# SHI-Labs/Versatile-Diffusion

Hardware: NVIDIA H100
Metric: 512x512 images/sec @ 50-step DDIM (bs=4/GPU) (higher is better)
Workload: dtype bf16

## Files before the change

### include/vdb200.h

```cpp
#ifndef VDB200_H_
#define VDB200_H_

#include <stddef.h>

#ifdef __cplusplus
extern "C" {
#endif

enum { VDB_OK = 0, VDB_ERR_INVALID = 1, VDB_ERR_CUDA = 2, VDB_ERR_UNSUPPORTED = 3 };
enum { VDB_ACT_NONE = 0, VDB_ACT_SILU = 1, VDB_ACT_GELU = 2, VDB_ACT_QUICK_GELU = 3, VDB_ACT_GEGLU = 4,
       VDB_ACT_GELU_TANH = 5 ,
       VDB_ACT_TANH = 6  };

const char* vdb_version(void);
const char* vdb_last_error(void);
long long vdb_launch_count(void);
void vdb_reset_launch_count(void);
int vdb_num_sms(void);

int vdb_ddim_cfg_step(const float* e_uncond, const float* e_cond, const float* x, const float* noise,
                      const float* coef, const int* step_idx, float scale, float temperature, float* x_prev,
                      float* x_prev_dup, float* pred_x0, long long n, void* stream);
int vdb_axpby_f32(const float* x, const float* z, float a, float b, float* y, long long n, void* stream);
int vdb_add_int(int* p, int delta, void* stream);
int vdb_lincomb4_f32(const float* x0, const float* x1, const float* x2, const float* x3, float c0, float c1, float c2,
                     float c3, float* y, long long n, void* stream);

int vdb_gemm_bf16(const void* A, long long M, long long K, long long lda, const void* A2, long long K2,
                  long long lda2, const void* W, long long N, long long ldw, const float* bias,
                  long long bias_bstride, long long rows_per_batch, const void* resid, long long ldr, void* out,
                  long long ldo, int out_f32, int act, float alpha, int bn, int ksplit, void* workspace,
                  size_t ws_bytes, void* stream);

int vdb_igemm_last_plan(int* out, int n);

int vdb_gemm_ln_bf16(const void* A, long long M, long long K, long long lda, const void* W, long long N, long long ldw,
                     const float* bias, const void* resid, long long ldr, void* out, long long ldo, int act,
                     const float* ln_stats, long long ln_rows, int ln_parts, int ln_dim, float ln_eps, const float* ln_colsum,
                     int ln_on_cols, const float* ln_rowbias, float* stats_out, int* stats_parts, int bn, void* stream);

int vdb_gemm_skinny_fits(int S, long long K);
int vdb_gemm_skinny_bf16(const void* small1, int S, long long K1, long long lds1, const void* small2, long long K2, long long lds2,
                         const void* big, long long R, long long ldb, const float* bias, long long bias_bstride,
                         const void* resid, long long ldr, void* out, long long ldo, int transpose_out, void* stream);

int vdb_conv3x3_bf16(const void* X, int B, int H, int W, int C, int mode, const void* Wt, int N, long long ldw,
                     const void* skip1, int Cs1, const void* skip2, int Cs2, const float* bias,
                     long long bias_bstride, const void* resid, long long ldr, void* out, long long ldo,
                     int out_f32, int act, int bn, int ksplit, void* workspace, size_t ws_bytes, void* stream);

int vdb_attention_dk_pad(int d_head);
int vdb_attention_dv_pad(int d_head);
int vdb_attention_bf16(const void* Q, long long ldq, int q_col0, const void* K, long long ldk, int k_col0,
                       const void* Vt, long long ldv, void* out, long long ldo, int B, int H, int Nq, int Nk,
                       int q_bstride, int kv_bstride, int d_head, float scale, int causal, void* stream);
int vdb_attention_varlen_bf16(const void* Q, long long ldq, int q_col0, const void* K, long long ldk, int k_col0,
                              const void* Vt, long long ldv, void* out, long long ldo, int B, int H, int Nq, int Nk,
                              int q_bstride, int kv_bstride, int d_head, float scale, int causal, const int* kv_len,
                              void* stream);

int vdb_groupnorm_nsplit(int B, int HW);
long long vdb_groupnorm_scratch_floats(int B, int HW);
int vdb_groupnorm_nhwc(const void* x1, int C1, const void* x2, int C2, int B, int HW, int groups, const float* gamma,
                       const float* beta, float eps, int act, float* scratch, void* y, void* stream);

int vdb_layernorm(const void* x, long long rows, int C, const float* gamma, const float* beta, float eps, void* y,
                  void* stream);

int vdb_norm_last_plan(int* out, int n);

int vdb_upsample2x_nhwc(const void* x, int B, int H, int W, int C, void* y, void* stream);

int vdb_clip_to_u8_hwc(const float* x, int n, int H, int W, void* y , void* stream);
int vdb_resample_h_u8(const void* x , int n, int H, int Win, int Wout, const int* bounds, const int* kk,
                      int ksize, void* y , void* stream);
int vdb_resample_v_crop_norm(const void* x , int n, int Hin, int W, const int* bounds, const int* kk,
                             int ksize , int top, int left, int S, const float* mean3,
                             const float* std3, float* y , void* stream);

int vdb_interleave2x2_nhwc(const void* src, int B, int H, int W, int C, void* y, void* stream);

int vdb_im2col3x3_small(const float* x, int B, int H, int W, int Cin, int Kpad, float in_scale, float in_shift,
                        void* y, void* stream);

int vdb_permute_f32(const float* x, int B, int C, long long HW, int to_nhwc, float mul, float add, int clamp01,
                    float* y, void* stream);
int vdb_gaussian_sample(const float* moments, const float* noise, int C, long long npix, float post_mul, float* z,
                        void* stream);
int vdb_cast_f32_bf16(const float* x, void* y, long long n, void* stream);
int vdb_pointwise_small(const float* x, long long npix, int Cin, int Cout, const float* Wm, const float* bias,
                        float pre_mul, float* y, void* stream);
int vdb_cast_bf16_f32(const void* x, float* y, long long n, void* stream);

int vdb_timestep_embedding(const long long* ts, const int* step_idx, int B, int dim, float neg_log_period,
                           float* out, void* stream);

int vdb_linear_small(const float* x, int M, int K, const void* Wt, int N, const float* bias, int act_in, int act_out,
                     float* out, void* stream);

int vdb_clip_text_embed(const long long* tokens, const float* tok_emb, const float* pos_emb, int B, int L, int Lp, int C,
                        void* x, void* stream);
int vdb_patchify(const float* pixels, int B, int Cin, int HW, int P, int Kpad, void* y, void* stream);
int vdb_vit_assemble(const void* patches, const float* cls, const float* pos, const float* tok_scale, int B, int L, int Lp,
                     int C, void* x, void* stream);
int vdb_scale_by_row_norm(const void* z, const int* idx, const float* row_scale, int B, int L, int Lp, int C, float* out,
                          void* stream);

int vdb_softmax_rows(const void* x, long long rows, int n, long long ld, float scale, void* y, void* stream);

int vdb_affine_act_rows(const void* x, long long rows, int n, const float* gamma, const float* beta, int act, void* y, void* stream);

int vdb_pack_conv_weight(const float* w, int Cout, int Cin, int kh, int kw, void* out, long long ldo, long long col0, void* stream);
int vdb_pack_geglu(const float* w, const float* b, int n2, int K, void* w_out, float* b_out, void* stream);
int vdb_pad_heads(const float* w, int H, int d, int dpad, int K, void* out, void* stream);

int vdb_textdec_gemv(const float* x, int R, long long K, long long ldx, const float* ln_gamma, const float* ln_beta, float ln_eps,
                     const void* W, long long N, long long ldw, const float* bias, int act, int accumulate, float* out, long long ldo,
                     void* stream);
int vdb_textdec_attention(const float* qkv, long long ldq, const float* mem, long long ldm, float* kcache, float* vcache, int R,
                          int H, int T, const int* step, float scale, float* out, long long ldo, void* stream);
int vdb_textdec_embed(const int* tokens, int ldt, const int* step, const float* wte, int V, const float* wpe, int P, int pos_offset,
                      const float* emb, int R, int D, float* h, void* stream);
int vdb_textdec_sample(const float* logits, int R, int V, long long ldl, float temperature, const unsigned long long* seed,
                       const double* uniforms, int ldu, const int* forced, int ldf, int* tokens, int ldt, int* done, int* lengths,
                       const int* step, int eos, int max_len, float* record, void* stream);

#ifdef __cplusplus
}
#endif
#endif
```

### versatile-diffusion_b200/csrc/common.cuh

```cuda
#pragma once
#include <cuda.h>
#include <cuda_bf16.h>
#include <cuda_runtime.h>
#include <stdint.h>

namespace vdb {

#define VDB_DEVINL __device__ __forceinline__

enum : int {
  VDB_OK = 0,
  VDB_ERR_INVALID = 1,
  VDB_ERR_CUDA = 2,
  VDB_ERR_UNSUPPORTED = 3,
};

VDB_DEVINL float4 lds_f4(uint32_t addr) {
  float4 v;
  asm volatile("ld.shared.v4.f32 {%0, %1, %2, %3}, [%4];" : "=f"(v.x), "=f"(v.y), "=f"(v.z), "=f"(v.w) : "r"(addr));
  return v;
}

VDB_DEVINL float2 lds_f2(uint32_t addr) {
  float2 v;
  asm volatile("ld.shared.v2.f32 {%0, %1}, [%2];" : "=f"(v.x), "=f"(v.y) : "r"(addr));
  return v;
}
VDB_DEVINL void stmatrix_x4(uint32_t addr, uint32_t r0, uint32_t r1, uint32_t r2, uint32_t r3) {
  asm volatile("stmatrix.sync.aligned.m8n8.x4.shared.b16 [%0], {%1, %2, %3, %4};" ::"r"(addr), "r"(r0), "r"(r1), "r"(r2), "r"(r3)
               : "memory");
}

VDB_DEVINL uint32_t smem_u32(const void* p) {
  return static_cast<uint32_t>(__cvta_generic_to_shared(p));
}

VDB_DEVINL uint32_t lane_id() {
  uint32_t l;
  asm volatile("mov.u32 %0, %%laneid;" : "=r"(l));
  return l;
}

VDB_DEVINL bool elect_one() {
  uint32_t pred = 0;
  asm volatile(
      "{\n\t"
      ".reg .pred P;\n\t"
      "elect.sync _|P, 0xffffffff;\n\t"
      "selp.u32 %0, 1, 0, P;\n\t"
      "}\n"
      : "=r"(pred));
  return pred != 0;
}

VDB_DEVINL void mbar_init(uint64_t* bar, uint32_t count) {
  asm volatile("mbarrier.init.shared::cta.b64 [%0], %1;" ::"r"(smem_u32(bar)), "r"(count));
}
VDB_DEVINL void fence_barrier_init() {
  asm volatile("fence.mbarrier_init.release.cluster;" ::: "memory");
}
VDB_DEVINL void fence_proxy_async_smem() {
  asm volatile("fence.proxy.async.shared::cta;" ::: "memory");
}
VDB_DEVINL void mbar_arrive_expect_tx(uint64_t* bar, uint32_t bytes) {
  asm volatile("mbarrier.arrive.expect_tx.shared::cta.b64 _, [%0], %1;" ::"r"(smem_u32(bar)),
               "r"(bytes)
               : "memory");
}
VDB_DEVINL void mbar_arrive(uint64_t* bar) {
  asm volatile("mbarrier.arrive.shared::cta.b64 _, [%0];" ::"r"(smem_u32(bar)) : "memory");
}
VDB_DEVINL bool mbar_try_wait(uint64_t* bar, uint32_t parity) {
  uint32_t ok;
  asm volatile(
      "{\n\t"
      ".reg .pred P;\n\t"
      "mbarrier.try_wait.parity.shared::cta.b64 P, [%1], %2;\n\t"
      "selp.u32 %0, 1, 0, P;\n\t"
      "}\n"
      : "=r"(ok)
      : "r"(smem_u32(bar)), "r"(parity)
      : "memory");
  return ok != 0;
}
VDB_DEVINL void mbar_wait(uint64_t* bar, uint32_t parity) {
  while (!mbar_try_wait(bar, parity)) {
  }
}

VDB_DEVINL void tma_prefetch_desc(const CUtensorMap* m) {
  asm volatile("prefetch.tensormap [%0];" ::"l"(reinterpret_cast<uint64_t>(m)) : "memory");
}
VDB_DEVINL void tma_load_2d(void* smem_dst, const CUtensorMap* m, uint64_t* bar, int c0, int c1) {
  asm volatile(
      "cp.async.bulk.tensor.2d.shared::cluster.global.tile.mbarrier::complete_tx::bytes"
      " [%0], [%1, {%3, %4}], [%2];" ::"r"(smem_u32(smem_dst)),
      "l"(reinterpret_cast<uint64_t>(m)), "r"(smem_u32(bar)), "r"(c0), "r"(c1)
      : "memory");
}
VDB_DEVINL void tma_load_4d(void* smem_dst, const CUtensorMap* m, uint64_t* bar, int c0, int c1,
                            int c2, int c3) {
  asm volatile(
      "cp.async.bulk.tensor.4d.shared::cluster.global.tile.mbarrier::complete_tx::bytes"
      " [%0], [%1, {%3, %4, %5, %6}], [%2];" ::"r"(smem_u32(smem_dst)),
      "l"(reinterpret_cast<uint64_t>(m)), "r"(smem_u32(bar)), "r"(c0), "r"(c1), "r"(c2), "r"(c3)
      : "memory");
}

VDB_DEVINL void tma_store_4d(const CUtensorMap* m, const void* smem_src, int c0, int c1, int c2, int c3) {
  asm volatile(
      "cp.async.bulk.tensor.4d.global.shared::cta.tile.bulk_group [%0, {%2, %3, %4, %5}], [%1];" ::"l"(
          reinterpret_cast<uint64_t>(m)),
      "r"(smem_u32(smem_src)), "r"(c0), "r"(c1), "r"(c2), "r"(c3)
      : "memory");
}
VDB_DEVINL void bulk_commit() { asm volatile("cp.async.bulk.commit_group;" ::: "memory"); }
template <int N>
VDB_DEVINL void bulk_wait_read() { asm volatile("cp.async.bulk.wait_group.read %0;" ::"n"(N) : "memory"); }
template <int N>
VDB_DEVINL void bulk_wait() { asm volatile("cp.async.bulk.wait_group %0;" ::"n"(N) : "memory"); }

VDB_DEVINL uint32_t cluster_ctarank() {
  uint32_t r;
  asm volatile("mov.u32 %0, %%cluster_ctarank;" : "=r"(r));
  return r;
}
VDB_DEVINL void cluster_sync_all() {
  asm volatile("barrier.cluster.arrive.release.aligned;\n\tbarrier.cluster.wait.acquire.aligned;" ::: "memory");
}
VDB_DEVINL uint32_t mapa_u32(uint32_t local_addr, uint32_t rank) {
  uint32_t r;
  asm volatile("mapa.shared::cluster.u32 %0, %1, %2;" : "=r"(r) : "r"(local_addr), "r"(rank));
  return r;
}
VDB_DEVINL void mbar_arrive_cluster(uint32_t cluster_addr) {
  asm volatile("mbarrier.arrive.release.cluster.shared::cluster.b64 _, [%0];" ::"r"(cluster_addr) : "memory");
}

VDB_DEVINL uint64_t make_desc_sw128(uint32_t smem_addr) {
  uint64_t d = 0;
  d |= static_cast<uint64_t>((smem_addr & 0x3FFFF) >> 4);
  d |= static_cast<uint64_t>(1) << 16;
  d |= static_cast<uint64_t>(1024 >> 4) << 32;
  d |= static_cast<uint64_t>(1) << 62;
  return d;
}
VDB_DEVINL void wgmma_fence() { asm volatile("wgmma.fence.sync.aligned;" ::: "memory"); }
VDB_DEVINL void wgmma_commit() { asm volatile("wgmma.commit_group.sync.aligned;" ::: "memory"); }
template <int N>
VDB_DEVINL void wgmma_wait() { asm volatile("wgmma.wait_group.sync.aligned %0;" ::"n"(N) : "memory"); }
template <int R>
VDB_DEVINL void wgmma_fence_regs(float (&d)[R]) {
#pragma unroll
  for (int i = 0; i < R; ++i) asm volatile("" : "+f"(d[i])::"memory");
}

VDB_DEVINL unsigned long long gtime() {
  unsigned long long t;
  asm volatile("mov.u64 %0, %%globaltimer;" : "=l"(t));
  return t;
}

VDB_DEVINL void pdl_wait() { asm volatile("griddepcontrol.wait;" ::: "memory"); }
VDB_DEVINL void pdl_launch_dependents() { asm volatile("griddepcontrol.launch_dependents;" ::: "memory"); }

VDB_DEVINL uint32_t pack_bf16x2(float lo, float hi) {
  __nv_bfloat162 v = __floats2bfloat162_rn(lo, hi);
  return *reinterpret_cast<uint32_t*>(&v);
}
VDB_DEVINL float2 unpack_bf16x2(uint32_t u) {
  __nv_bfloat162 v = *reinterpret_cast<__nv_bfloat162*>(&u);
  return __bfloat1622float2(v);
}
VDB_DEVINL float ex2_mufu(float x) {
  float y;
  asm("ex2.approx.ftz.f32 %0, %1;" : "=f"(y) : "f"(x));
  return y;
}
VDB_DEVINL float ex2_poly(float x) {
  x = fmaxf(x, -126.0f);
  const float r = x + 12582912.0f;
  const float f = x - (r - 12582912.0f);
  float p = fmaf(0.0550886838f, f, 0.242604051f);
  p = fmaf(p, f, 0.693276242f);
  p = fmaf(p, f, 0.99992894f);
  return __int_as_float(__float_as_int(p) + (__float_as_int(r) << 23));
}
VDB_DEVINL float silu_f(float x) { return __fdividef(x, 1.0f + __expf(-x)); }
VDB_DEVINL float silu_bf16_f(float x) {
  float th;
  asm("tanh.approx.f32 %0, %1;" : "=f"(th) : "f"(0.5f * x));
  const float hx = 0.5f * x;
  return fmaf(hx, th, hx);
}
VDB_DEVINL float gelu_erf_f(float x) { return 0.5f * x * (1.0f + erff(x * 0.70710678118654752f)); }
VDB_DEVINL float gelu_as_f(float x) {
  const float z = fabsf(x) * 0.70710678118654752f;
  const float t = __fdividef(1.0f, fmaf(0.3275911f, z, 1.0f));
  float poly = fmaf(1.061405429f, t, -1.453152027f);
  poly = fmaf(poly, t, 1.421413741f);
  poly = fmaf(poly, t, -0.284496736f);
  poly = fmaf(poly, t, 0.254829592f);
  const float erf_abs = 1.0f - poly * t * __expf(-z * z);
  return 0.5f * x * (1.0f + copysignf(erf_abs, x));
}
VDB_DEVINL float gelu_fast_f(float x) {
  const float u = x * fmaf(0.0356774081f, x * x, 0.7978845608f);
  float th;
  asm("tanh.approx.f32 %0, %1;" : "=f"(th) : "f"(u));
  const float hx = 0.5f * x;
  return fmaf(hx, th, hx);
}
VDB_DEVINL float quick_gelu_f(float x) { return __fdividef(x, 1.0f + __expf(-1.702f * x)); }

}

#include "wgmma.cuh"
```

### versatile-diffusion_b200/csrc/igemm.cu

```cuda
#include "common.cuh"
#include "host_util.h"

namespace vdb {

constexpr int kBlockM = 128;
constexpr int kBlockK = 64;
constexpr int kMaxA = 6;
constexpr int kMaxSeg = 12;
constexpr uint32_t kABytes = kBlockM * kBlockK * 2;

struct ASeg {
  int16_t tmap;
  int16_t dw;
  int16_t dh;
  int16_t nkb;
  int32_t c0;
};

struct alignas(64) IgemmParams {
  CUtensorMap tmA[kMaxA];
  CUtensorMap tmB;
  CUtensorMap tmO;
  ASeg seg[kMaxSeg];
  int nseg;
  int kb_total;
  int ksplit;
  int kb_per_split;
  int TW, TH, TB;
  int Wo, Ho, Bo;
  int tilesW, tilesH, tilesB, tilesN;
  int N;
  const float* bias;
  long long bias_bstride;
  int rows_per_batch;
  const __nv_bfloat16* resid;
  long long ldr;
  void* out;
  long long ldo;
  int out_f32;
  int act;
  float alpha;
  float* partial;
  const float* ln_stats;
  long long ln_mstat;
  int ln_parts;
  int ln_on_cols;
  float ln_inv_dim, ln_eps;
  const float* ln_colsum;
  const float* ln_rowbias;
  float* stats_out;
  int epi_alt;
  int nfast;
  unsigned long long* timeline;
  unsigned smem_bytes;
  int chunked;
};

enum { ACT_NONE = 0, ACT_SILU = 1, ACT_GELU = 2, ACT_QGELU = 3, ACT_GEGLU = 4 };

#ifdef VDB_TIMELINE
#define VDB_TL(slot, it) do { if (p.timeline && blockIdx.x == 0 && (it) < 8) p.timeline[(it) * 16 + (slot)] = gtime(); } while (0)
#define VDB_TLE(slot, it) do { if (warp == 0 && lane == 0) VDB_TL(slot, it); } while (0)
#else
#define VDB_TL(slot, it) do { } while (0)
#define VDB_TLE(slot, it) do { } while (0)
#endif

VDB_DEVINL float apply_act(float v, int act) {
  switch (act) {
    case ACT_SILU: return silu_f(v);
    case ACT_GELU: return gelu_erf_f(v);
    case ACT_QGELU: return quick_gelu_f(v);
    default: return v;
  }
}

template <int BN, int STAGES, int EW, int MODE>
__global__ void __launch_bounds__(32 + 32 * EW, 1) igemm_kernel(const __grid_constant__ IgemmParams p) {
  constexpr bool kTmaEpi = MODE >= 3;
  constexpr bool kGegluEpi = MODE == 4 || MODE == 6;
  constexpr bool kLnIn = MODE == 5 || MODE == 6;
  constexpr bool kStatsOut = MODE == 7;
  constexpr int kNumEpiWarps = EW;
  constexpr int kNumEpiThreads = EW * 32;
  constexpr int kWPQ = EW / 4;
  static_assert(EW == 8, "two consumer warpgroups of 64 rows each");
  constexpr uint32_t kBBytes = BN * kBlockK * 2;
  constexpr uint32_t kStageBytes = kABytes + kBBytes;
  constexpr int kAccStride = BN + 4;
  constexpr uint32_t kRingBytes = STAGES * kStageBytes;
  constexpr uint32_t kAccBytes = kBlockM * kAccStride * 4;
  constexpr uint32_t kRegion = kRingBytes > kAccBytes ? kRingBytes : kAccBytes;
  static_assert(kBBytes % 1024 == 0, "B stage must keep 1024B alignment");
  static_assert(BN % 32 == 0 && BN >= 32 && BN <= 256, "invalid wgmma N");

  extern __shared__ __align__(1024) uint8_t smem_raw[];
  uint8_t* smem = reinterpret_cast<uint8_t*>((reinterpret_cast<uintptr_t>(smem_raw) + 1023) & ~uintptr_t(1023));
  uint8_t* smemA = smem;
  uint8_t* smemB = smem + STAGES * kABytes;
  float* sacc = reinterpret_cast<float*>(smem);
  float* sstage = reinterpret_cast<float*>(smem + kRegion);
  uint64_t* full_bar = reinterpret_cast<uint64_t*>(smem + kRegion + EW * 4096);
  uint64_t* empty_bar = full_bar + STAGES;
  uint64_t* acc_free = empty_bar + STAGES;
  float* sbias = reinterpret_cast<float*>(acc_free + 2);
  float* slnx = sbias + BN;
  const uint32_t sbias_s = smem_u32(sbias), slnx_s = smem_u32(slnx);
  (void)slnx_s;
  if constexpr (kLnIn) {
    if (reinterpret_cast<uint8_t*>(slnx + BN) > smem_raw + p.smem_bytes) __trap();
  }
  auto epi_bar_sync = [] { asm volatile("bar.sync 1, %0;" ::"n"(EW * 32) : "memory"); };

  const int warp = threadIdx.x >> 5;
  const int lane = threadIdx.x & 31;

  if (warp == EW && lane == 0) {
    for (int i = 0; i < kMaxA; ++i) tma_prefetch_desc(&p.tmA[i]);
    tma_prefetch_desc(&p.tmB);
    if constexpr (MODE >= 3) tma_prefetch_desc(&p.tmO);
  }
  if (threadIdx.x == 0) {
    for (int s = 0; s < STAGES; ++s) {
      mbar_init(&full_bar[s], 1);
      mbar_init(&empty_bar[s], kNumEpiWarps);
    }
    mbar_init(acc_free, kNumEpiWarps);
    fence_barrier_init();
  }
  __syncthreads();
  pdl_launch_dependents();
  pdl_wait();

  const int tilesM = p.tilesW * p.tilesH * p.tilesB;
  const int unitsM = tilesM;
  const int num_tiles = unitsM * p.tilesN * p.ksplit;
  const int n_ctas = gridDim.x, cta_id = blockIdx.x;
  const int per_cta = (num_tiles + n_ctas - 1) / n_ctas;
  const int t_first = p.chunked ? cta_id * per_cta : cta_id, t_step = p.chunked ? 1 : n_ctas;
  const int t_end = p.chunked ? min(num_tiles, t_first + per_cta) : num_tiles;

  if (warp == EW) {
    if (lane == 0) {
      uint32_t stage = 0, phase = 0;
      const bool flat = (p.tilesH == 1) && (p.tilesB == 1);
      const int step_m = t_step % unitsM, step_r = t_step / unitsM;
      int unit_m = t_first % unitsM, rest = t_first / unitsM;
      const int nf_step_n = p.nfast ? t_step % p.tilesN : 0, nf_step_m = p.nfast ? t_step / p.tilesN : 0;
      int nf_n = p.nfast ? t_first % p.tilesN : 0, nf_m = p.nfast ? t_first / p.tilesN : 0;
      int it = 0;
      for (int t = t_first; t < t_end; t += t_step, ++it) {
        const int m_idx = p.nfast ? nf_m : unit_m;
        int n_idx = p.nfast ? nf_n : rest, ks = 0;
        if (p.ksplit > 1) { n_idx = rest % p.tilesN; ks = rest / p.tilesN; }
        nf_n += nf_step_n; nf_m += nf_step_m;
        if (p.nfast && nf_n >= p.tilesN) { nf_n -= p.tilesN; ++nf_m; }
        int wt = m_idx, ht = 0, bt = 0;
        if (!flat) {
          wt = m_idx % p.tilesW;
          const int q = m_idx / p.tilesW;
          ht = q % p.tilesH;
          bt = q / p.tilesH;
        }
        unit_m += step_m; rest += step_r;
        if (unit_m >= unitsM) { unit_m -= unitsM; ++rest; }
        const int w0 = wt * p.TW, h0 = ht * p.TH, b0 = bt * p.TB;
        const int n0 = n_idx * BN;
        const int kb_begin = ks * p.kb_per_split;
        const int kb_end = min(p.kb_total, kb_begin + p.kb_per_split);
        int kb = 0;
        if (!kTmaEpi && it > 0) mbar_wait(acc_free, (it - 1) & 1);
        VDB_TL(0, it);
        for (int s = 0; s < p.nseg; ++s) {
          const ASeg sg = p.seg[s];
          if (kb + sg.nkb <= kb_begin) { kb += sg.nkb; continue; }
          for (int j = 0; j < sg.nkb; ++j, ++kb) {
            if (kb < kb_begin) continue;
            if (kb >= kb_end) break;
            mbar_wait(&empty_bar[stage], phase ^ 1);
            mbar_arrive_expect_tx(&full_bar[stage], kStageBytes);
            tma_load_4d(smemA + stage * kABytes, &p.tmA[sg.tmap], &full_bar[stage],
                        sg.c0 + j * kBlockK, w0 + sg.dw, h0 + sg.dh, b0);
            tma_load_2d(smemB + stage * kBBytes, &p.tmB, &full_bar[stage], kb * kBlockK, n0);
            if (++stage == STAGES) { stage = 0; phase ^= 1; }
          }
          if (kb >= kb_end) break;
        }
      }
    }
  } else {
    const int quarter = warp & 3;
    const int half = warp >> 2;
    const int r = quarter * 32 + lane;
    const int tr_row = lane >> 2, tr_q = lane & 3;
    float* stage = sstage + warp * 1024;
    const uint32_t sacc_row = smem_u32(sacc) + static_cast<uint32_t>(r * kAccStride * 4);
    auto acc_ld32 = [&](int col, uint32_t (&v)[32]) {
#pragma unroll
      for (int i = 0; i < 8; ++i) {
        const float4 x = lds_f4(sacc_row + (col + 4 * i) * 4);
        v[4 * i] = __float_as_uint(x.x); v[4 * i + 1] = __float_as_uint(x.y);
        v[4 * i + 2] = __float_as_uint(x.z); v[4 * i + 3] = __float_as_uint(x.w);
      }
    };
    uint32_t ml_stage = 0, ml_phase = 0;
    float acc[BN / 2];
    auto mainloop = [&](int kb_begin, int kb_end) {
      const int g = warp >> 2;
#pragma unroll
      for (int i = 0; i < BN / 2; ++i) acc[i] = 0.f;
      uint32_t prev = 0;
      for (int kb = kb_begin; kb < kb_end; ++kb) {
        mbar_wait(&full_bar[ml_stage], ml_phase);
        wgmma_fence();
        const uint64_t adesc = make_desc_sw128(smem_u32(smemA + ml_stage * kABytes + g * (64 * 128)));
        const uint64_t bdesc = make_desc_sw128(smem_u32(smemB + ml_stage * kBBytes));
#pragma unroll
        for (int k = 0; k < kBlockK / 16; ++k) wgmma_ss<BN>(acc, adesc + 2 * k, bdesc + 2 * k, (kb > kb_begin || k > 0) ? 1u : 0u);
        wgmma_commit();
        if (kb > kb_begin) {
          wgmma_wait<1>();
          __syncwarp();
          if (lane == 0) mbar_arrive(&empty_bar[prev]);
        }
        prev = ml_stage;
        if (++ml_stage == STAGES) { ml_stage = 0; ml_phase ^= 1; }
      }
      wgmma_wait<0>();
      wgmma_fence_regs(acc);
      __syncwarp();
      if (lane == 0 && kb_end > kb_begin) mbar_arrive(&empty_bar[prev]);
      if constexpr (!kTmaEpi) {
        epi_bar_sync();
        float* srow = sacc + (g * 64 + (warp & 3) * 16 + (lane >> 2)) * kAccStride + 2 * (lane & 3);
#pragma unroll
        for (int j = 0; j < BN / 8; ++j) {
          *reinterpret_cast<float2*>(srow + 8 * j) = make_float2(acc[4 * j], acc[4 * j + 1]);
          *reinterpret_cast<float2*>(srow + 8 * kAccStride + 8 * j) = make_float2(acc[4 * j + 2], acc[4 * j + 3]);
        }
        epi_bar_sync();
      }
    };
    auto stage_write = [&](const uint32_t (&v)[32]) {
      float* srow = stage + lane * 32;
#pragma unroll
      for (int j = 0; j < 8; ++j)
        *reinterpret_cast<uint4*>(srow + ((j ^ (lane & 7)) << 2)) = make_uint4(v[4 * j], v[4 * j + 1], v[4 * j + 2], v[4 * j + 3]);
    };
    auto stage_read = [&](int k, float (&o)[8]) {
      const int row = k * 8 + tr_row;
      const float* srow = stage + row * 32;
      const float4 x0 = *reinterpret_cast<const float4*>(srow + (((2 * tr_q) ^ (row & 7)) << 2));
      const float4 x1 = *reinterpret_cast<const float4*>(srow + (((2 * tr_q + 1) ^ (row & 7)) << 2));
      o[0] = x0.x; o[1] = x0.y; o[2] = x0.z; o[3] = x0.w; o[4] = x1.x; o[5] = x1.y; o[6] = x1.z; o[7] = x1.w;
    };
    int it = 0;
    int st_buf = 0;
    (void)st_buf;
    const float* sbias_src = nullptr;
    const int tw = r % p.TW;
    const int th = (r / p.TW) % p.TH;
    const int tb = r / (p.TW * p.TH);
    const bool flat = (p.tilesH == 1) && (p.tilesB == 1);
    const int step_m = t_step % unitsM, step_r = t_step / unitsM;
    int unit_m = t_first % unitsM, rest = t_first / unitsM;
    const int nf_step_n = p.nfast ? t_step % p.tilesN : 0, nf_step_m = p.nfast ? t_step / p.tilesN : 0;
    int nf_n = p.nfast ? t_first % p.tilesN : 0, nf_m = p.nfast ? t_first / p.tilesN : 0;
    const int e_row0 = (warp >> 2) * 64 + (warp & 3) * 16;
    int e_tw[2], e_th[2], e_tb[2];
#pragma unroll
    for (int h = 0; h < 2; ++h) {
      const int er = e_row0 + (lane >> 2) + 8 * h;
      e_tw[h] = er % p.TW; e_th[h] = (er / p.TW) % p.TH; e_tb[h] = er / (p.TW * p.TH);
    }
    constexpr int kLnPre = 8;
    float2 ln_pre[kLnIn ? kLnPre : 1];
    auto ln_prefetch = [&](int row) {
      if constexpr (kLnIn) {
        const bool ok = row < p.Wo;
        const int i0 = (lane >> 4) * kLnPre;
#pragma unroll
        for (int i = 0; i < kLnPre; ++i)
          ln_pre[i] = (ok && i0 + i < p.ln_parts)
                          ? __ldg(reinterpret_cast<const float2*>(p.ln_stats) + static_cast<long long>(i0 + i) * p.ln_mstat + row)
                          : make_float2(0.f, 0.f);
      }
    };
    if constexpr (kLnIn) {
      if (!p.ln_on_cols && p.ln_parts <= 2 * kLnPre && t_first < t_end) ln_prefetch((t_first % unitsM) * kBlockM + e_row0 + (lane & 15));
    }
    for (int t = t_first; t < t_end; t += t_step, ++it) {
      const int m_idx = p.nfast ? nf_m : unit_m;
      int n_idx = p.nfast ? nf_n : rest, ks = 0;
      if (p.ksplit > 1) { n_idx = rest % p.tilesN; ks = rest / p.tilesN; }
      nf_n += nf_step_n; nf_m += nf_step_m;
      if (p.nfast && nf_n >= p.tilesN) { nf_n -= p.tilesN; ++nf_m; }
      int wt = m_idx, ht = 0, bt = 0;
      if (!flat) {
        wt = m_idx % p.tilesW;
        const int q = m_idx / p.tilesW;
        ht = q % p.tilesH;
        bt = q / p.tilesH;
      }
      unit_m += step_m; rest += step_r;
      if (unit_m >= unitsM) { unit_m -= unitsM; ++rest; }
      const int w = wt * p.TW + tw, h = ht * p.TH + th, b = bt * p.TB + tb;
      const bool row_ok = (w < p.Wo) && (h < p.Ho) && (b < p.Bo);
      const int gp = (b * p.Ho + h) * p.Wo + w;
      const int gp_first = ((bt * p.TB) * p.Ho + ht * p.TH) * p.Wo + wt * p.TW;
      const int n0 = n_idx * BN;

      int gp_k[4];
      bool ok_k[4];
      if constexpr (!kTmaEpi) {
        const unsigned okmask = __ballot_sync(0xffffffffu, row_ok);
#pragma unroll
        for (int k = 0; k < 4; ++k) {
          const int src = k * 8 + tr_row;
          gp_k[k] = __shfl_sync(0xffffffffu, gp, src);
          ok_k[k] = (okmask >> src) & 1u;
        }
      }
      const int gp_last = ((bt * p.TB + p.TB - 1) * p.Ho + ht * p.TH + p.TH - 1) * p.Wo + wt * p.TW + p.TW - 1;
      const bool bias_uniform = (MODE != 0) ? (p.bias != nullptr)
                                            : (p.bias && p.ksplit == 1 &&
                                               (p.bias_bstride == 0 || gp_first / p.rows_per_batch == gp_last / p.rows_per_batch));
      if constexpr (kLnIn) {
        const float* key = reinterpret_cast<const float*>(static_cast<uintptr_t>(n0) + 1);
        if (key != sbias_src) {
          epi_bar_sync();
          for (int i = threadIdx.x; i < BN; i += kNumEpiThreads) {
            const int n = n0 + i;
            float a = 0.f, b = 0.f;
            if (n < p.N) {
              if (p.ln_on_cols) {
                float su = 0.f, sq = 0.f;
#pragma unroll 8
                for (int ch = 0; ch < p.ln_parts; ++ch) {
                  const float2 v = __ldg(reinterpret_cast<const float2*>(p.ln_stats) + static_cast<long long>(ch) * p.ln_mstat + n);
                  su += v.x; sq += v.y;
                }
                const float mu = su * p.ln_inv_dim;
                a = mu;
                b = rsqrtf(fmaxf(sq * p.ln_inv_dim - mu * mu, 0.f) + p.ln_eps);
              } else {
                a = __ldg(p.ln_colsum + n);
                b = p.bias ? __ldg(p.bias + n) : 0.f;
              }
            }
            slnx[i] = a;
            sbias[i] = b;
          }
          epi_bar_sync();
          sbias_src = key;
        }
      } else if (bias_uniform) {
        const float* brow = p.bias + (p.bias_bstride ? static_cast<long long>(gp_first / p.rows_per_batch) * p.bias_bstride : 0) + n0;
        if (brow != sbias_src) {
          epi_bar_sync();
          for (int i = threadIdx.x; i < BN; i += kNumEpiThreads) sbias[i] = (n0 + i < p.N) ? __ldg(brow + i) : 0.f;
          epi_bar_sync();
          sbias_src = brow;
        }
      }
      const float* bias_g = (p.bias && !bias_uniform)
                                ? p.bias + (p.bias_bstride ? static_cast<long long>(gp / p.rows_per_batch) * p.bias_bstride : 0) : nullptr;

      const int f_nchunks = min(BN / 32, (p.N - n0) / 32);
      const bool has_resid = p.resid != nullptr;
      const int f_first = (((BN / 32) % kWPQ) != 0) ? ((half + it) % kWPQ) : half;
      auto load_resid_fast = [&](int c, uint4 (&rr)[4]) {
#pragma unroll
        for (int k = 0; k < 4; ++k)
          if (ok_k[k]) rr[k] = __ldg(reinterpret_cast<const uint4*>(p.resid + static_cast<long long>(gp_k[k]) * p.ldr + n0 + c * 32 + tr_q * 8));
      };
      uint4 rr_first[4];
      if constexpr (MODE == 1) {
        if (has_resid && f_first < f_nchunks) load_resid_fast(f_first, rr_first);
      }

      int e_gp[2];
      bool e_ok[2];
#pragma unroll
      for (int h = 0; h < 2; ++h) {
        const int ew = wt * p.TW + e_tw[h], eh = ht * p.TH + e_th[h], eb = bt * p.TB + e_tb[h];
        e_ok[h] = (ew < p.Wo) && (eh < p.Ho) && (eb < p.Bo);
        e_gp[h] = (eb * p.Ho + eh) * p.Wo + ew;
      }
      float ln_a0[2] = {0.f, 0.f}, ln_a1[2] = {1.f, 1.f};
      if constexpr (kLnIn) {
        if (p.ln_on_cols) {
#pragma unroll
          for (int h = 0; h < 2; ++h) {
            if (e_ok[h]) {
              ln_a0[h] = __ldg(p.ln_colsum + e_gp[h]);
              ln_a1[h] = p.ln_rowbias ? __ldg(p.ln_rowbias + e_gp[h]) : 0.f;
            }
          }
        } else {
          float su = 0.f, sq = 0.f;
          if (p.ln_parts <= 2 * kLnPre) {
#pragma unroll
            for (int i = 0; i < kLnPre; ++i) { su += ln_pre[i].x; sq += ln_pre[i].y; }
#pragma unroll
            for (int i = 0; i < kLnPre; ++i) {
              su += __shfl_sync(0xffffffffu, ln_pre[i].x, lane | 16);
              sq += __shfl_sync(0xffffffffu, ln_pre[i].y, lane | 16);
            }
          } else {
            const int row = m_idx * kBlockM + e_row0 + (lane & 15);
            if (row < p.Wo) {
#pragma unroll 8
              for (int ch = 0; ch < p.ln_parts; ++ch) {
                const float2 v = __ldg(reinterpret_cast<const float2*>(p.ln_stats) + static_cast<long long>(ch) * p.ln_mstat + row);
                su += v.x; sq += v.y;
              }
            }
          }
          const float mu = su * p.ln_inv_dim;
          const float rs = rsqrtf(fmaxf(sq * p.ln_inv_dim - mu * mu, 0.f) + p.ln_eps);
#pragma unroll
          for (int h = 0; h < 2; ++h) {
            ln_a0[h] = __shfl_sync(0xffffffffu, mu, (lane >> 2) + 8 * h);
            ln_a1[h] = __shfl_sync(0xffffffffu, rs, (lane >> 2) + 8 * h);
          }
        }
        if (!p.ln_on_cols && p.ln_parts <= 2 * kLnPre && t + t_step < t_end) ln_prefetch(unit_m * kBlockM + e_row0 + (lane & 15));
      }
      VDB_TLE(4, it);
      mainloop(ks * p.kb_per_split, min(p.kb_total, ks * p.kb_per_split + p.kb_per_split));
      VDB_TLE(5, it);

      auto geglu_tile = [&] {
        constexpr int HALF = BN / 2;
        const int nout0 = n_idx * HALF;
        const int Nout = p.N / 2;
#pragma unroll 1
        for (int c = (((HALF / 32) % kWPQ) != 0) ? ((half + it) % kWPQ) : half; c < HALF / 32; c += kWPQ) {
          uint32_t v[32];
          float a[4][8];
          acc_ld32(c * 32, v);
          stage_write(v);
          __syncwarp();
#pragma unroll
          for (int k = 0; k < 4; ++k) stage_read(k, a[k]);
          __syncwarp();
          acc_ld32(HALF + c * 32, v);
          stage_write(v);
          __syncwarp();
          float bv[8], bg[8];
#pragma unroll
          for (int i = 0; i < 8; ++i) {
            bv[i] = p.bias ? sbias[c * 32 + tr_q * 8 + i] : 0.f;
            bg[i] = p.bias ? sbias[HALF + c * 32 + tr_q * 8 + i] : 0.f;
          }
#pragma unroll
          for (int k = 0; k < 4; ++k) {
            float g[8];
            stage_read(k, g);
            if (ok_k[k] && nout0 + c * 32 + tr_q * 8 + 7 < Nout) {
              float o[8];
#pragma unroll
              for (int i = 0; i < 8; ++i) o[i] = (a[k][i] + bv[i]) * gelu_fast_f(g[i] + bg[i]);
              *reinterpret_cast<uint4*>(reinterpret_cast<__nv_bfloat16*>(p.out) + static_cast<long long>(gp_k[k]) * p.ldo + nout0 + c * 32 + tr_q * 8) =
                  make_uint4(pack_bf16x2(o[0], o[1]), pack_bf16x2(o[2], o[3]), pack_bf16x2(o[4], o[5]), pack_bf16x2(o[6], o[7]));
            }
          }
          __syncwarp();
        }
      };
      if constexpr (kTmaEpi) {
        const uint32_t stg_s = smem_u32(sstage) + warp * 4096;
        const int ow = wt * p.TW + (e_row0 % p.TW), oh = ht * p.TH + ((e_row0 / p.TW) % p.TH), ob = bt * p.TB + e_row0 / (p.TW * p.TH);
        constexpr int OUTC = kGegluEpi ? BN / 2 : BN;
        const int ochunks = kGegluEpi ? OUTC / 32 : f_nchunks;
        const int ocol0 = n_idx * OUTC;
        const int tq2 = 2 * (lane & 3);
        const bool do_resid = (MODE == 3 || MODE == 7) && has_resid;
        const uint32_t* rrow[2];
#pragma unroll
        for (int h = 0; h < 2; ++h)
          rrow[h] = (do_resid && e_ok[h]) ? reinterpret_cast<const uint32_t*>(p.resid + static_cast<long long>(e_gp[h]) * p.ldr + ocol0 + tq2)
                                          : nullptr;
        auto load_resid = [&](int c, uint32_t (&rr)[2][4]) {
#pragma unroll
          for (int h = 0; h < 2; ++h)
#pragma unroll
            for (int jj = 0; jj < 4; ++jj) rr[h][jj] = rrow[h] ? __ldg(rrow[h] + (c * 32 + 8 * jj) / 2) : 0u;
        };
        uint32_t rr[2][4];
        if (do_resid) load_resid(0, rr);
        float st_su[2][2] = {{0.f, 0.f}, {0.f, 0.f}}, st_sq[2][2] = {{0.f, 0.f}, {0.f, 0.f}};
        (void)st_su; (void)st_sq;
        float nrm[2];
#pragma unroll
        for (int h = 0; h < 2; ++h) nrm[h] = -ln_a1[h] * ln_a0[h];
        (void)nrm;
#pragma unroll
        for (int c = 0; c < OUTC / 32; ++c) {
          if (c >= ochunks) break;
          float o[4][2][2];
#pragma unroll
          for (int jj = 0; jj < 4; ++jj) {
            const int n = c * 32 + 8 * jj + tq2;
            const float* va = acc + 4 * (4 * c + jj);
            if constexpr (kGegluEpi) {
              const float* vg = acc + 4 * (BN / 16 + 4 * c + jj);
              if constexpr (kLnIn) {
                const float2 sa = lds_f2(slnx_s + 4 * n), ca = lds_f2(sbias_s + 4 * n);
                const float2 sg = lds_f2(slnx_s + 4 * (OUTC + n)), cg = lds_f2(sbias_s + 4 * (OUTC + n));
#pragma unroll
                for (int h = 0; h < 2; ++h) {
                  o[jj][h][0] = fmaf(ln_a1[h], va[2 * h], fmaf(nrm[h], sa.x, ca.x)) * gelu_fast_f(fmaf(ln_a1[h], vg[2 * h], fmaf(nrm[h], sg.x, cg.x)));
                  o[jj][h][1] = fmaf(ln_a1[h], va[2 * h + 1], fmaf(nrm[h], sa.y, ca.y)) * gelu_fast_f(fmaf(ln_a1[h], vg[2 * h + 1], fmaf(nrm[h], sg.y, cg.y)));
                }
              } else {
                const float2 ba = p.bias ? lds_f2(sbias_s + 4 * n) : make_float2(0.f, 0.f);
                const float2 bg = p.bias ? lds_f2(sbias_s + 4 * (OUTC + n)) : make_float2(0.f, 0.f);
#pragma unroll
                for (int h = 0; h < 2; ++h) {
                  o[jj][h][0] = (va[2 * h] + ba.x) * gelu_fast_f(vg[2 * h] + bg.x);
                  o[jj][h][1] = (va[2 * h + 1] + ba.y) * gelu_fast_f(vg[2 * h + 1] + bg.y);
                }
              }
            } else if constexpr (kLnIn) {
              if (p.ln_on_cols) {
                const float2 mu = lds_f2(slnx_s + 4 * n), rs = lds_f2(sbias_s + 4 * n);
#pragma unroll
                for (int h = 0; h < 2; ++h) {
                  o[jj][h][0] = fmaf(rs.x, fmaf(mu.x, -ln_a0[h], va[2 * h]), ln_a1[h]);
                  o[jj][h][1] = fmaf(rs.y, fmaf(mu.y, -ln_a0[h], va[2 * h + 1]), ln_a1[h]);
                }
              } else {
                const float2 sx = lds_f2(slnx_s + 4 * n), cx = lds_f2(sbias_s + 4 * n);
#pragma unroll
                for (int h = 0; h < 2; ++h) {
                  o[jj][h][0] = fmaf(ln_a1[h], va[2 * h], fmaf(nrm[h], sx.x, cx.x));
                  o[jj][h][1] = fmaf(ln_a1[h], va[2 * h + 1], fmaf(nrm[h], sx.y, cx.y));
                }
              }
            } else {
              const float2 bb = p.bias ? lds_f2(sbias_s + 4 * n) : make_float2(0.f, 0.f);
#pragma unroll
              for (int h = 0; h < 2; ++h) {
                o[jj][h][0] = va[2 * h] + bb.x;
                o[jj][h][1] = va[2 * h + 1] + bb.y;
              }
            }
          }
          if (do_resid) {
            uint32_t rn[2][4];
            const bool more = c + 1 < ochunks;
            if (more) load_resid(c + 1, rn);
#pragma unroll
            for (int h = 0; h < 2; ++h)
#pragma unroll
              for (int jj = 0; jj < 4; ++jj) {
                const float2 x = unpack_bf16x2(rr[h][jj]);
                o[jj][h][0] += x.x;
                o[jj][h][1] += x.y;
              }
            if (more) {
#pragma unroll
              for (int h = 0; h < 2; ++h)
#pragma unroll
                for (int jj = 0; jj < 4; ++jj) rr[h][jj] = rn[h][jj];
            }
          }
          if constexpr (kStatsOut) {
#pragma unroll
            for (int h = 0; h < 2; ++h)
#pragma unroll
              for (int jj = 0; jj < 4; ++jj)
#pragma unroll
                for (int e = 0; e < 2; ++e) {
                  st_su[h][c & 1] += o[jj][h][e];
                  st_sq[h][c & 1] = fmaf(o[jj][h][e], o[jj][h][e], st_sq[h][c & 1]);
                }
          }
          if (lane == 0) bulk_wait_read<3>();
          __syncwarp();
          const uint32_t box = stg_s + st_buf * 1024;
          {
            const int mi = lane >> 3, brow = (mi & 1) * 8 + (lane & 7);
#pragma unroll
            for (int u = 0; u < 2; ++u) {
              const int unit = 2 * u + (mi >> 1);
              stmatrix_x4(box + brow * 64 + ((unit ^ ((brow >> 1) & 3)) << 4),
                          pack_bf16x2(o[2 * u][0][0], o[2 * u][0][1]), pack_bf16x2(o[2 * u][1][0], o[2 * u][1][1]),
                          pack_bf16x2(o[2 * u + 1][0][0], o[2 * u + 1][0][1]), pack_bf16x2(o[2 * u + 1][1][0], o[2 * u + 1][1][1]));
            }
          }
          fence_proxy_async_smem();
          __syncwarp();
          if (lane == 0) {
            tma_store_4d(&p.tmO, reinterpret_cast<const uint8_t*>(sstage) + warp * 4096 + st_buf * 1024, ocol0 + c * 32, ow, oh, ob);
            bulk_commit();
          }
          st_buf = (st_buf + 1) & 3;
        }
        if constexpr (kStatsOut) {
#pragma unroll
          for (int h = 0; h < 2; ++h)
#pragma unroll
            for (int par = 0; par < 2; ++par) {
              float su = st_su[h][par], sq = st_sq[h][par];
              su += __shfl_xor_sync(0xffffffffu, su, 1); sq += __shfl_xor_sync(0xffffffffu, sq, 1);
              su += __shfl_xor_sync(0xffffffffu, su, 2); sq += __shfl_xor_sync(0xffffffffu, sq, 2);
              if ((lane & 3) == 0 && e_ok[h])
                reinterpret_cast<float2*>(p.stats_out)[static_cast<long long>(n_idx * 2 + par) * (static_cast<long long>(p.Bo) * p.Ho * p.Wo) + e_gp[h]] =
                    make_float2(su, sq);
            }
        }
      } else if constexpr (MODE == 1) {
        uint4 rr[4];
#pragma unroll
        for (int k = 0; k < 4; ++k) rr[k] = rr_first[k];
#pragma unroll 1
        for (int c = f_first; c < f_nchunks; c += kWPQ) {
          uint32_t v[32];
          acc_ld32(c * 32, v);
          uint4 rn[4];
          if (has_resid && c + kWPQ < f_nchunks) load_resid_fast(c + kWPQ, rn);
          stage_write(v);
          __syncwarp();
          float bb[8];
#pragma unroll
          for (int i = 0; i < 8; ++i) bb[i] = p.bias ? sbias[c * 32 + tr_q * 8 + i] : 0.f;
#pragma unroll
          for (int k = 0; k < 4; ++k) {
            float o[8];
            stage_read(k, o);
            if (ok_k[k]) {
#pragma unroll
              for (int i = 0; i < 8; ++i) o[i] += bb[i];
              if (has_resid) {
                const uint32_t w4[4] = {rr[k].x, rr[k].y, rr[k].z, rr[k].w};
#pragma unroll
                for (int q = 0; q < 4; ++q) {
                  const float2 x = unpack_bf16x2(w4[q]);
                  o[2 * q] += x.x;
                  o[2 * q + 1] += x.y;
                }
              }
              *reinterpret_cast<uint4*>(reinterpret_cast<__nv_bfloat16*>(p.out) + static_cast<long long>(gp_k[k]) * p.ldo + n0 + c * 32 + tr_q * 8) =
                  make_uint4(pack_bf16x2(o[0], o[1]), pack_bf16x2(o[2], o[3]), pack_bf16x2(o[4], o[5]), pack_bf16x2(o[6], o[7]));
            }
          }
          __syncwarp();
#pragma unroll
          for (int k = 0; k < 4; ++k) rr[k] = rn[k];
        }
      } else if constexpr (MODE == 2) {
        geglu_tile();
      } else if (p.ksplit > 1) {
        const long long Mtot = static_cast<long long>(p.Bo) * p.Ho * p.Wo;
        float* dst = p.partial + (static_cast<long long>(ks) * Mtot + gp) * p.N + n0;
#pragma unroll 1
        for (int c = half; c < BN / 32; c += kWPQ) {
          if (n0 + c * 32 >= p.N) break;
          uint32_t v[32];
          acc_ld32(c * 32, v);
          if (row_ok) {
#pragma unroll
            for (int j = 0; j < 32; j += 4) {
              const int n = n0 + c * 32 + j;
              if (n + 3 < p.N) {
                *reinterpret_cast<float4*>(dst + c * 32 + j) =
                    make_float4(__uint_as_float(v[j]), __uint_as_float(v[j + 1]),
                                __uint_as_float(v[j + 2]), __uint_as_float(v[j + 3]));
              } else {
                for (int q = 0; q < 4; ++q)
                  if (n + q < p.N) dst[c * 32 + j + q] = __uint_as_float(v[j + q]);
              }
            }
          }
        }
      } else if (p.act == ACT_GEGLU) {
        geglu_tile();
      } else {
        const int nchunks = min(BN / 32, (p.N - n0 + 31) / 32);
        auto chunk = [&](int c, const uint32_t (&v)[32], const uint4 (&rr)[4], bool fast) {
          const int nb = n0 + c * 32;
          if (fast) {
            stage_write(v);
            __syncwarp();
            if (c == half) VDB_TLE(8, it);
            float bb[8];
#pragma unroll
            for (int i = 0; i < 8; ++i) bb[i] = p.bias ? sbias[c * 32 + tr_q * 8 + i] : 0.f;
#pragma unroll
            for (int k = 0; k < 4; ++k) {
              float o[8];
              stage_read(k, o);
              if (ok_k[k]) {
#pragma unroll
                for (int i = 0; i < 8; ++i) o[i] += bb[i];
                if (p.alpha != 1.f) {
#pragma unroll
                  for (int i = 0; i < 8; ++i) o[i] *= p.alpha;
                }
                if (p.act != ACT_NONE) {
#pragma unroll
                  for (int i = 0; i < 8; ++i) o[i] = apply_act(o[i], p.act);
                }
                if (p.resid) {
                  const uint32_t w4[4] = {rr[k].x, rr[k].y, rr[k].z, rr[k].w};
#pragma unroll
                  for (int q = 0; q < 4; ++q) {
                    const float2 x = unpack_bf16x2(w4[q]);
                    o[2 * q] += x.x;
                    o[2 * q + 1] += x.y;
                  }
                }
                *reinterpret_cast<uint4*>(reinterpret_cast<__nv_bfloat16*>(p.out) + static_cast<long long>(gp_k[k]) * p.ldo + nb + tr_q * 8) =
                    make_uint4(pack_bf16x2(o[0], o[1]), pack_bf16x2(o[2], o[3]), pack_bf16x2(o[4], o[5]), pack_bf16x2(o[6], o[7]));
              }
              if (c == half && k == 0) VDB_TLE(9, it);
            }
            __syncwarp();
            if (c == half) VDB_TLE(10, it);
          } else if (row_ok) {
            float f[32];
#pragma unroll
            for (int j = 0; j < 32; ++j) f[j] = __uint_as_float(v[j]);
            if (p.bias) {
#pragma unroll
              for (int j = 0; j < 32; ++j)
                if (nb + j < p.N) f[j] += bias_uniform ? sbias[c * 32 + j] : __ldg(bias_g + nb + j);
            }
#pragma unroll
            for (int j = 0; j < 32; ++j) f[j] = apply_act(f[j] * p.alpha, p.act);
            if (p.resid) {
              const __nv_bfloat16* rs = p.resid + static_cast<long long>(gp) * p.ldr + nb;
#pragma unroll
              for (int j = 0; j < 32; ++j) if (nb + j < p.N) f[j] += __bfloat162float(rs[j]);
            }
            if (p.out_f32) {
              float* dst = reinterpret_cast<float*>(p.out) + static_cast<long long>(gp) * p.ldo + nb;
#pragma unroll
              for (int j = 0; j < 32; ++j) if (nb + j < p.N) dst[j] = f[j];
            } else {
              __nv_bfloat16* dst = reinterpret_cast<__nv_bfloat16*>(p.out) + static_cast<long long>(gp) * p.ldo + nb;
#pragma unroll
              for (int j = 0; j < 32; ++j) if (nb + j < p.N) dst[j] = __float2bfloat16(f[j]);
            }
          }
        };
        auto is_fast = [&](int c) { return (n0 + c * 32 + 32 <= p.N) && !p.out_f32 && (bias_uniform || !p.bias); };
        auto load_resid = [&](int c, uint4 (&rr)[4]) {
          if (p.resid && is_fast(c)) {
#pragma unroll
            for (int k = 0; k < 4; ++k)
              if (ok_k[k]) rr[k] = __ldg(reinterpret_cast<const uint4*>(p.resid + static_cast<long long>(gp_k[k]) * p.ldr + n0 + c * 32 + tr_q * 8));
          }
        };
        const int first = (p.epi_alt && ((BN / 32) % kWPQ) != 0) ? ((half + it) % kWPQ) : half;
#pragma unroll 1
        for (int c = first; c < nchunks; c += kWPQ) {
          uint4 rr[4];
          load_resid(c, rr);
          uint32_t v[32];
          acc_ld32(c * 32, v);
          if (c == first) VDB_TLE(7, it);
          chunk(c, v, rr, is_fast(c));
        }
      }
      if constexpr (!kTmaEpi) {
        fence_proxy_async_smem();
        __syncwarp();
        VDB_TLE(6, it);
        if (lane == 0) mbar_arrive(acc_free);
      }
    }
    if constexpr (MODE >= 3) {
      if (lane == 0) bulk_wait<0>();
    }
  }
}

__global__ void splitk_reduce_kernel(const float* __restrict__ partial, int ksplit, long long M, int N,
                                     const float* __restrict__ bias, long long bias_bstride, int rows_per_batch,
                                     const __nv_bfloat16* __restrict__ resid, long long ldr, void* out,
                                     long long ldo, int out_f32, int act, float alpha) {
  pdl_launch_dependents();
  pdl_wait();
  const long long total = M * (N / 4);
  for (long long i = blockIdx.x * static_cast<long long>(blockDim.x) + threadIdx.x; i < total;
       i += static_cast<long long>(gridDim.x) * blockDim.x) {
    const long long m = i / (N / 4);
    const int n = static_cast<int>(i % (N / 4)) * 4;
    float4 acc = make_float4(0.f, 0.f, 0.f, 0.f);
    for (int s = 0; s < ksplit; ++s) {
      const float4 v = __ldg(reinterpret_cast<const float4*>(partial + (static_cast<long long>(s) * M + m) * N + n));
      acc.x += v.x; acc.y += v.y; acc.z += v.z; acc.w += v.w;
    }
    float f[4] = {acc.x, acc.y, acc.z, acc.w};
    if (bias) {
      const float* bp = bias + (bias_bstride ? (m / rows_per_batch) * bias_bstride : 0) + n;
      for (int q = 0; q < 4; ++q) f[q] += __ldg(bp + q);
    }
    for (int q = 0; q < 4; ++q) f[q] *= alpha;
    for (int q = 0; q < 4; ++q) f[q] = apply_act(f[q], act);
    if (resid) {
      for (int q = 0; q < 4; ++q) f[q] += __bfloat162float(resid[m * ldr + n + q]);
    }
    if (out_f32) {
      *reinterpret_cast<float4*>(reinterpret_cast<float*>(out) + m * ldo + n) = make_float4(f[0], f[1], f[2], f[3]);
    } else {
      uint2 o = make_uint2(pack_bf16x2(f[0], f[1]), pack_bf16x2(f[2], f[3]));
      *reinterpret_cast<uint2*>(reinterpret_cast<__nv_bfloat16*>(out) + m * ldo + n) = o;
    }
  }
}

template <int BN, int STAGES, int EW, int MODE>
static int launch_igemm(const IgemmParams& p0, int num_units, cudaStream_t stream) {
  constexpr bool kLn = MODE == 5 || MODE == 6;
  constexpr size_t ring = STAGES * (kABytes + BN * kBlockK * 2), acc = kBlockM * (BN + 4) * 4;
  constexpr size_t need = (ring > acc ? ring : acc) + (2 * STAGES + 2) * 8 + BN * 4 + (kLn ? BN * 4 : 0) + EW * 4096;
  constexpr size_t smem = (need + 1024 <= 227 * 1024) ? need + 1024 : 227 * 1024;
  static_assert(need + 896 <= 227 * 1024, "igemm shared-memory budget");
  constexpr int threads = 32 + 32 * EW;
  IgemmParams p = p0;
  p.smem_bytes = static_cast<unsigned>(smem);
  static bool configured = false;
  if (!configured) {
    VDB_CUDA_CHECK(cudaFuncSetAttribute(igemm_kernel<BN, STAGES, EW, MODE>, cudaFuncAttributeMaxDynamicSharedMemorySize,
                                        static_cast<int>(smem)));
    prefer_max_smem(igemm_kernel<BN, STAGES, EW, MODE>);
    configured = true;
  }
  const int grid = std::min(num_units, num_sms());
  VDB_CUDA_CHECK(launch_pdl(igemm_kernel<BN, STAGES, EW, MODE>, dim3(grid), dim3(threads), smem, stream, p));
  count_launch();
  return VDB_OK;
}

static int pick_bn(int N, int act, int forced) {
  if (forced) return forced;
  if (act == ACT_GEGLU) return 256;
  if (N <= 64) return 64;
  if (N % 256 == 0) return 256;
  if (N % 160 == 0) return 160;
  if (N % 128 == 0) return 128;
  if (N <= 128) return 128;
  if (N <= 160) return 160;
  return 256;
}

static unsigned long long* g_timeline = nullptr;

constexpr int kPlanFields = 9;
static thread_local int g_last_plan[kPlanFields] = {0};

static int check_epilogue_pointers(const void* out, long long ldo, int out_f32, const void* resid, long long ldr, const char* who) {
  if ((reinterpret_cast<uintptr_t>(out) & 15) || (resid && (reinterpret_cast<uintptr_t>(resid) & 15)))
    return set_error(VDB_ERR_INVALID, "%s: out and resid must be 16-byte aligned", who);
  if (!out_f32 && (ldo % 8)) return set_error(VDB_ERR_INVALID, "%s: ldo must be a multiple of 8 for bf16 out", who);
  if (resid && (ldr % 8)) return set_error(VDB_ERR_INVALID, "%s: ldr must be a multiple of 8", who);
  return VDB_OK;
}

struct IgemmEpilogue {
  const float* bias = nullptr;
  long long bias_bstride = 0;
  int rows_per_batch = 1;
  const void* resid = nullptr;
  long long ldr = 0;
  void* out = nullptr;
  long long ldo = 0;
  int out_f32 = 0;
  int act = 0;
  float alpha = 1.f;
  const float* ln_stats = nullptr;
  long long ln_mstat = 0;
  int ln_parts = 0;
  int ln_dim = 0;
  float ln_eps = 0.f;
  const float* ln_colsum = nullptr;
  int ln_on_cols = 0;
  const float* ln_rowbias = nullptr;
  float* stats_out = nullptr;
  int* stats_parts = nullptr;
  int out_parity = -1;
};

static int run_igemm(IgemmParams& p, const void* Wt, long long N, long long Ktot, long long ldw,
                     const IgemmEpilogue& e, int bn_forced, int ksplit_forced, void* workspace,
                     size_t ws_bytes, cudaStream_t stream) {
  const bool ln_in = e.ln_stats != nullptr, st_out = e.stats_out != nullptr;
  if (ln_in || st_out) ksplit_forced = 1;
  int BN = pick_bn(static_cast<int>(N), e.act, bn_forced);
  static const int bn_model = [] { const char* ev = getenv("VDB_BN_MODEL"); return (ev && ev[0] == '0') ? 0 : 1; }();
  if (bn_model && !bn_forced && e.act != ACT_GEGLU && p.kb_total >= 8) {
    const long long tm = static_cast<long long>(p.tilesW) * p.tilesH * p.tilesB;
    const int cand[4] = {256, 160, 128, 64};
    double best = 1e30;
    for (int c : cand) {
      const long long tiles = tm * ((N + c - 1) / c);
      long long ks = 1;
      if (ksplit_forced > 0) ks = ksplit_forced;
      else if (tiles * 2 <= num_sms() && p.kb_total >= 16 && (N % 4) == 0 && workspace)
        ks = std::max<long long>(1, std::min<long long>(std::min<long long>(num_sms() / tiles, p.kb_total / 8), 16));
      const long long waves = (tiles * ks + num_sms() - 1) / num_sms();
      const double per_kb = std::max(2.0 * c, (16384.0 + 128.0 * c) / 90.0);
      const double kb_unit = static_cast<double>((p.kb_total + ks - 1) / ks);
      const double cost = static_cast<double>(waves) * (kb_unit * per_kb + 1500.0) + (ks > 1 ? 12000.0 : 0.0);
      if (cost < best * 0.97) { best = cost; BN = c; }
    }
  }
  if (!bn_forced && !bn_model && e.act != ACT_GEGLU && p.kb_total < 32) {
    const int tm = p.tilesW * p.tilesH * p.tilesB;
    auto tiles = [&](int bn) { return tm * static_cast<int>((N + bn - 1) / bn); };
    while (BN > 64 && tiles(BN) * 2 <= num_sms()) BN = (BN == 256) ? 160 : (BN == 160 ? 128 : 64);
  }
  if (BN != 64 && BN != 128 && BN != 160 && BN != 256) return set_error(VDB_ERR_INVALID, "igemm: bad BN");
  if (e.act == ACT_GEGLU && (N % BN) != 0) return set_error(VDB_ERR_INVALID, "igemm: GEGLU needs N % 256 == 0");
  p.N = static_cast<int>(N);
  p.tilesN = static_cast<int>((N + BN - 1) / BN);
  p.bias = e.bias; p.bias_bstride = e.bias_bstride; p.rows_per_batch = e.rows_per_batch > 0 ? e.rows_per_batch : 1;
  p.resid = reinterpret_cast<const __nv_bfloat16*>(e.resid); p.ldr = e.ldr;
  p.out = e.out; p.ldo = e.ldo; p.out_f32 = e.out_f32; p.act = e.act; p.alpha = e.alpha;
  const long long M = static_cast<long long>(p.Bo) * p.Ho * p.Wo;
  if (M >= (1LL << 30)) return set_error(VDB_ERR_UNSUPPORTED, "igemm: more than 2^30 output rows");
  const int tilesM = p.tilesW * p.tilesH * p.tilesB;
  const int mn_tiles = tilesM * p.tilesN;
  int ksplit = 1;
  if (ksplit_forced > 0) {
    ksplit = ksplit_forced;
  } else if (e.act != ACT_GEGLU && mn_tiles * 2 <= num_sms() && p.kb_total >= 16 && (N % 4) == 0) {
    ksplit = std::min(std::min(num_sms() / mn_tiles, p.kb_total / 8), 16);
    if (ksplit < 1) ksplit = 1;
  }
  if (ksplit > 1) {
    const size_t need = static_cast<size_t>(ksplit) * M * N * sizeof(float);
    if (workspace == nullptr || ws_bytes < need || e.act == ACT_GEGLU || (N % 4) || (e.out_f32 && (e.ldo % 4))) ksplit = 1;
  }
  p.ksplit = ksplit;
  p.kb_per_split = (p.kb_total + ksplit - 1) / ksplit;
  p.ksplit = (p.kb_total + p.kb_per_split - 1) / p.kb_per_split;
  p.partial = reinterpret_cast<float*>(workspace);
  p.ln_stats = e.ln_stats; p.ln_mstat = e.ln_mstat; p.ln_parts = e.ln_parts; p.ln_on_cols = e.ln_on_cols;
  if (e.stats_parts) *e.stats_parts = 2 * p.tilesN;
  p.ln_inv_dim = e.ln_dim > 0 ? 1.f / static_cast<float>(e.ln_dim) : 0.f; p.ln_eps = e.ln_eps;
  p.ln_colsum = e.ln_colsum; p.ln_rowbias = e.ln_rowbias; p.stats_out = e.stats_out;
  p.timeline = g_timeline;
  static const int epi_alt = [] { const char* ev = getenv("VDB_EPI_ALT"); return (ev && ev[0] == '0') ? 0 : 1; }();
  p.epi_alt = epi_alt;
  static const int nfast_mode = [] { const char* ev = getenv("VDB_NFAST"); return ev ? atoi(ev) : 0; }();
  {
    const int grid = std::min(mn_tiles * p.ksplit, num_sms());
    const double a_bytes = static_cast<double>(M) * static_cast<double>(Ktot) * 2.0;
    p.nfast = (nfast_mode != 0 && p.ksplit == 1 && p.tilesN > 1 && (grid % p.tilesN) == 0 &&
               (nfast_mode == 2 || a_bytes > 48e6) && !ln_in) ? 1 : 0;
  }
  {
    static const int chunked_mode = [] { const char* ev = getenv("VDB_CHUNKED"); return ev ? atoi(ev) : 0; }();
    const long long units = static_cast<long long>(tilesM) * p.tilesN * p.ksplit;
    const int grid = static_cast<int>(std::min<long long>(units, num_sms()));
    p.chunked = (chunked_mode != 0 && !p.nfast && p.ksplit == 1 && p.tilesN > 1 && units >= 3LL * grid) ? 1 : 0;
  }
  int rc = make_tmap_2d(&p.tmB, Wt, static_cast<uint64_t>(Ktot), static_cast<uint64_t>(N),
                        static_cast<uint64_t>(ldw) * 2, kBlockK, BN);
  if (rc) return rc;
  const int num_tiles = mn_tiles * p.ksplit;
  static const int spec = [] { const char* ev = getenv("VDB_IGEMM_SPEC"); return (ev && ev[0] == '0') ? 0 : 1; }();
  int mode = 0;
  const bool one_bias_row = e.bias == nullptr || e.bias_bstride == 0 ||
                            (p.TB == 1 && (static_cast<long long>(p.Ho) * p.Wo == p.rows_per_batch ||
                                           (p.Ho == 1 && p.Bo == 1 && p.rows_per_batch % kBlockM == 0)));
  if (spec && p.ksplit == 1 && !e.out_f32 && one_bias_row) {
    if (e.act == ACT_GEGLU && BN == 256) mode = 2;
    else if (e.act == ACT_NONE && e.alpha == 1.f && (N % 32) == 0) mode = 1;
  }
  static const int epi_tma = [] { const char* ev = getenv("VDB_EPI_TMA"); return (ev && ev[0] == '0') ? 0 : 1; }();
  if (epi_tma && (mode == 1 || mode == 2) && (reinterpret_cast<uintptr_t>(e.out) & 15) == 0 &&
      (!e.resid || (reinterpret_cast<uintptr_t>(e.resid) & 15) == 0)) {
    const int bw = std::min(p.TW, 16), bh = std::min(p.TH, 16 / bw), bb = 16 / (bw * bh);
    const long long ncols = (mode == 2) ? N / 2 : N;
    const int py = e.out_parity >= 0 ? (e.out_parity >> 1) : 0, px = e.out_parity >= 0 ? (e.out_parity & 1) : 0;
    const uint64_t il = e.out_parity >= 0 ? 2 : 1;
    const void* obase = reinterpret_cast<const __nv_bfloat16*>(e.out) + (static_cast<long long>(py) * (il * p.Wo) + px) * e.ldo;
    if (bb <= p.TB &&
        make_tmap_4d_sw64(&p.tmO, obase, static_cast<uint64_t>(ncols), static_cast<uint64_t>(p.Wo), static_cast<uint64_t>(p.Ho),
                          static_cast<uint64_t>(p.Bo), il * static_cast<uint64_t>(e.ldo) * 2,
                          il * il * static_cast<uint64_t>(p.Wo) * e.ldo * 2,
                          il * il * static_cast<uint64_t>(p.Ho) * p.Wo * e.ldo * 2, 32, bw, bh, bb) == 0)
      mode += 2;
  }
  if (e.out_parity >= 0 && mode != 3)
    return set_error(VDB_ERR_UNSUPPORTED, "igemm: the interleaved-output upsample modes need the TMA-store epilogue (bf16 out, no "
                                          "activation, N %% 32 == 0, aligned out, VDB_EPI_TMA != 0)");
  if (ln_in || st_out) {
    if (ln_in && st_out) return set_error(VDB_ERR_UNSUPPORTED, "igemm: a launch either consumes or produces LayerNorm statistics");
    if (mode != 3 && !(mode == 4 && ln_in))
      return set_error(VDB_ERR_UNSUPPORTED, "igemm: LayerNorm statistics need the TMA-store epilogue (bf16 out, no activation or "
                                            "GEGLU, alpha 1, N %% 32 == 0, 16-byte aligned out / resid, VDB_EPI_TMA != 0)");
    if (ln_in && e.resid) return set_error(VDB_ERR_UNSUPPORTED, "igemm: a folded-LayerNorm GEMM takes no residual");
    if (ln_in && mode == 4 && e.ln_on_cols) return set_error(VDB_ERR_UNSUPPORTED, "igemm: GEGLU with column statistics");
    mode = st_out ? 7 : mode + 2;
  }
  {
    const int stages = BN == 64 ? 8 : BN == 128 ? 6 : BN == 160 ? 5 : 4;
    const int plan[kPlanFields] = {BN, stages, mode, p.ksplit, std::min(num_tiles, num_sms()), tilesM, p.tilesN, p.nfast, p.chunked};
    for (int i = 0; i < kPlanFields; ++i) g_last_plan[i] = plan[i];
  }
  if (mode == 7) {
    switch (BN) {
      case 64: rc = launch_igemm<64, 8, 8, 7>(p, num_tiles, stream); break;
      case 128: rc = launch_igemm<128, 6, 8, 7>(p, num_tiles, stream); break;
      case 160: rc = launch_igemm<160, 5, 8, 7>(p, num_tiles, stream); break;
      default: rc = launch_igemm<256, 4, 8, 7>(p, num_tiles, stream); break;
    }
  } else if (mode == 6) {
    rc = launch_igemm<256, 4, 8, 6>(p, num_tiles, stream);
  } else if (mode == 5) {
    switch (BN) {
      case 64: rc = launch_igemm<64, 8, 8, 5>(p, num_tiles, stream); break;
      case 128: rc = launch_igemm<128, 6, 8, 5>(p, num_tiles, stream); break;
      case 160: rc = launch_igemm<160, 5, 8, 5>(p, num_tiles, stream); break;
      default: rc = launch_igemm<256, 4, 8, 5>(p, num_tiles, stream); break;
    }
  } else if (mode == 4) {
    rc = launch_igemm<256, 4, 8, 4>(p, num_tiles, stream);
  } else if (mode == 3) {
    switch (BN) {
      case 64: rc = launch_igemm<64, 8, 8, 3>(p, num_tiles, stream); break;
      case 128: rc = launch_igemm<128, 6, 8, 3>(p, num_tiles, stream); break;
      case 160: rc = launch_igemm<160, 5, 8, 3>(p, num_tiles, stream); break;
      default: rc = launch_igemm<256, 4, 8, 3>(p, num_tiles, stream); break;
    }
  } else if (mode == 2) {
    rc = launch_igemm<256, 4, 8, 2>(p, num_tiles, stream);
  } else if (mode == 1) {
    switch (BN) {
      case 64: rc = launch_igemm<64, 8, 8, 1>(p, num_tiles, stream); break;
      case 128: rc = launch_igemm<128, 6, 8, 1>(p, num_tiles, stream); break;
      case 160: rc = launch_igemm<160, 5, 8, 1>(p, num_tiles, stream); break;
      default: rc = launch_igemm<256, 4, 8, 1>(p, num_tiles, stream); break;
    }
  } else {
    switch (BN) {
      case 64: rc = launch_igemm<64, 8, 8, 0>(p, num_tiles, stream); break;
      case 128: rc = launch_igemm<128, 6, 8, 0>(p, num_tiles, stream); break;
      case 160: rc = launch_igemm<160, 5, 8, 0>(p, num_tiles, stream); break;
      default: rc = launch_igemm<256, 4, 8, 0>(p, num_tiles, stream); break;
    }
  }
  if (rc) return rc;
  if (p.ksplit > 1) {
    const long long total = M * (N / 4);
    const int threads = 256;
    const int blocks = static_cast<int>(std::min<long long>((total + threads - 1) / threads, num_sms() * 8LL));
    VDB_PREFER_MAX_SMEM(splitk_reduce_kernel);
    VDB_CUDA_CHECK(launch_pdl(splitk_reduce_kernel, dim3(blocks), dim3(threads), 0, stream, (const float*)p.partial,
                              p.ksplit, M, static_cast<int>(N), p.bias, p.bias_bstride, p.rows_per_batch, p.resid,
                              p.ldr, p.out, p.ldo, p.out_f32, p.act, p.alpha));
    count_launch();
  }
  return VDB_OK;
}

static int pow2_ceil(int v) { int t = 1; while (t < v) t <<= 1; return t; }

static void set_tile_shape(IgemmParams& p, int Wo, int Ho, int Bo) {
  p.Wo = Wo; p.Ho = Ho; p.Bo = Bo;
  const int TW = std::min(pow2_ceil(Wo), 128);
  const int TH = std::min(pow2_ceil(Ho), 128 / TW);
  const int TB = 128 / (TW * TH);
  p.TW = TW; p.TH = TH; p.TB = TB;
  p.tilesW = (Wo + TW - 1) / TW;
  p.tilesH = (Ho + TH - 1) / TH;
  p.tilesB = (Bo + TB - 1) / TB;
}

}

using namespace vdb;

extern "C" {

void vdb_debug_igemm_timeline(void* buf) { g_timeline = reinterpret_cast<unsigned long long*>(buf); }

int vdb_igemm_last_plan(int* out, int n) {
  for (int i = 0; out && i < n && i < kPlanFields; ++i) out[i] = g_last_plan[i];
  return kPlanFields;
}

int vdb_gemm_bf16(const void* A, long long M, long long K, long long lda, const void* A2, long long K2,
                  long long lda2, const void* W, long long N, long long ldw, const float* bias,
                  long long bias_bstride, long long rows_per_batch, const void* resid, long long ldr, void* out,
                  long long ldo, int out_f32, int act, float alpha, int bn, int ksplit, void* workspace,
                  size_t ws_bytes, void* stream) {
  if (!A || !W || !out || M <= 0 || N <= 0 || K <= 0) return set_error(VDB_ERR_INVALID, "gemm: null/empty argument");
  if ((K % 8) || (lda % 8) || (ldw % 8)) return set_error(VDB_ERR_INVALID, "gemm: K, lda, ldw must be multiples of 8");
  if (A2 && ((K % kBlockK) || (K2 % 8) || (lda2 % 8)))
    return set_error(VDB_ERR_INVALID, "gemm: two-source A needs K % 64 == 0 and K2, lda2 % 8 == 0");
  if (M > 0x7fffffffLL || N > 0x7fffffffLL) return set_error(VDB_ERR_INVALID, "gemm: dimension too large");
  int rc = check_epilogue_pointers(out, ldo, out_f32, resid, ldr, "gemm");
  if (rc) return rc;
  IgemmParams p;
  memset(&p, 0, sizeof(p));
  p.Wo = static_cast<int>(M); p.Ho = 1; p.Bo = 1;
  p.TW = kBlockM; p.TH = 1; p.TB = 1;
  p.tilesW = static_cast<int>((M + kBlockM - 1) / kBlockM); p.tilesH = 1; p.tilesB = 1;
  rc = make_tmap_4d(&p.tmA[0], A, K, M, 1, 1, lda * 2, lda * 2 * M, lda * 2 * M, kBlockK, p.TW, 1, 1);
  if (rc) return rc;
  p.seg[0] = ASeg{0, 0, 0, static_cast<int16_t>((K + kBlockK - 1) / kBlockK), 0};
  p.nseg = 1;
  p.kb_total = p.seg[0].nkb;
  if (A2) {
    rc = make_tmap_4d(&p.tmA[1], A2, K2, M, 1, 1, lda2 * 2, lda2 * 2 * M, lda2 * 2 * M, kBlockK, p.TW, 1, 1);
    if (rc) return rc;
    p.seg[1] = ASeg{1, 0, 0, static_cast<int16_t>((K2 + kBlockK - 1) / kBlockK), 0};
    p.nseg = 2;
    p.kb_total += p.seg[1].nkb;
  }
  for (int i = p.nseg; i < kMaxA; ++i) p.tmA[i] = p.tmA[0];
  IgemmEpilogue e;
  e.bias = bias; e.bias_bstride = bias_bstride; e.rows_per_batch = static_cast<int>(rows_per_batch);
  e.resid = resid; e.ldr = ldr; e.out = out; e.ldo = ldo; e.out_f32 = out_f32; e.act = act; e.alpha = alpha;
  return run_igemm(p, W, N, K + (A2 ? K2 : 0), ldw, e, bn, ksplit, workspace, ws_bytes,
                   reinterpret_cast<cudaStream_t>(stream));
}

int vdb_gemm_ln_bf16(const void* A, long long M, long long K, long long lda, const void* W, long long N, long long ldw,
                     const float* bias, const void* resid, long long ldr, void* out, long long ldo, int act,
                     const float* ln_stats, long long ln_rows, int ln_parts, int ln_dim, float ln_eps, const float* ln_colsum,
                     int ln_on_cols, const float* ln_rowbias, float* stats_out, int* stats_parts, int bn, void* stream) {
  if (!A || !W || !out || M <= 0 || N <= 0 || K <= 0) return set_error(VDB_ERR_INVALID, "gemm_ln: null/empty argument");
  if ((K % 8) || (lda % 8) || (ldw % 8)) return set_error(VDB_ERR_INVALID, "gemm_ln: K, lda, ldw must be multiples of 8");
  if (M > 0x7fffffffLL || N > 0x7fffffffLL) return set_error(VDB_ERR_INVALID, "gemm_ln: dimension too large");
  if (!ln_stats && !stats_out) return set_error(VDB_ERR_INVALID, "gemm_ln: neither ln_stats nor stats_out given (use vdb_gemm_bf16)");
  if (ln_stats) {
    if (!ln_colsum || ln_dim <= 0 || ln_dim != K || ln_parts <= 0)
      return set_error(VDB_ERR_INVALID, "gemm_ln: need ln_colsum, ln_parts > 0 and ln_dim == K");
    if (ln_rows < (ln_on_cols ? N : M)) return set_error(VDB_ERR_INVALID, "gemm_ln: statistics table has too few rows");
  }
  if (stats_out && ((N % 32) || !stats_parts)) return set_error(VDB_ERR_INVALID, "gemm_ln: stats_out needs N %% 32 == 0 and stats_parts");
  int rc = check_epilogue_pointers(out, ldo, 0, resid, ldr, "gemm_ln");
  if (rc) return rc;
  IgemmParams p;
  memset(&p, 0, sizeof(p));
  p.Wo = static_cast<int>(M); p.Ho = 1; p.Bo = 1;
  p.TW = kBlockM; p.TH = 1; p.TB = 1;
  p.tilesW = static_cast<int>((M + kBlockM - 1) / kBlockM); p.tilesH = 1; p.tilesB = 1;
  rc = make_tmap_4d(&p.tmA[0], A, K, M, 1, 1, lda * 2, lda * 2 * M, lda * 2 * M, kBlockK, p.TW, 1, 1);
  if (rc) return rc;
  p.seg[0] = ASeg{0, 0, 0, static_cast<int16_t>((K + kBlockK - 1) / kBlockK), 0};
  p.nseg = 1;
  p.kb_total = p.seg[0].nkb;
  for (int i = p.nseg; i < kMaxA; ++i) p.tmA[i] = p.tmA[0];
  IgemmEpilogue e;
  e.bias = bias; e.resid = resid; e.ldr = ldr; e.out = out; e.ldo = ldo; e.act = act;
  e.ln_stats = ln_stats; e.ln_mstat = ln_rows; e.ln_parts = ln_parts; e.ln_dim = ln_dim; e.ln_eps = ln_eps; e.ln_colsum = ln_colsum;
  e.ln_on_cols = ln_on_cols; e.ln_rowbias = ln_rowbias; e.stats_out = stats_out; e.stats_parts = stats_parts;
  return run_igemm(p, W, N, K, ldw, e, bn, 1, nullptr, 0, reinterpret_cast<cudaStream_t>(stream));
}

int vdb_conv3x3_bf16(const void* X, int B, int H, int Wd, int C, int mode, const void* Wt, int N, long long ldw,
                     const void* skip1, int Cs1, const void* skip2, int Cs2, const float* bias,
                     long long bias_bstride, const void* resid, long long ldr, void* out, long long ldo,
                     int out_f32, int act, int bn, int ksplit, void* workspace, size_t ws_bytes, void* stream) {
  if (!X || !Wt || !out || B <= 0 || H <= 0 || Wd <= 0 || C <= 0 || N <= 0)
    return set_error(VDB_ERR_INVALID, "conv3x3: null/empty argument");
  if ((C % kBlockK) || (ldw % 8)) return set_error(VDB_ERR_INVALID, "conv3x3: C must be a multiple of 64, ldw of 8");
  if ((skip1 && (Cs1 % kBlockK)) || (skip2 && (Cs2 % kBlockK)))
    return set_error(VDB_ERR_INVALID, "conv3x3: skip channels must be multiples of 64");
  if (mode < 0 || mode > 10) return set_error(VDB_ERR_INVALID, "conv3x3: bad mode");
  const int out_parity = mode >= 7 ? mode - 7 : -1;
  if (mode >= 7) mode -= 4;
  if (out_parity >= 0 && (resid || out_f32 || ksplit > 1)) return set_error(VDB_ERR_INVALID, "conv3x3: modes 7..10 take no residual, bf16 out, no split-K");
  if (out_parity >= 0) ksplit = 1;
  const bool strided = (mode == 1 || mode == 2), folded = mode >= 3;
  if (strided && ((H & 1) || (Wd & 1))) return set_error(VDB_ERR_UNSUPPORTED, "conv3x3: stride 2 needs even H, W");
  if (folded && (skip1 || skip2)) return set_error(VDB_ERR_INVALID, "conv3x3: the folded-upsample modes take no skip inputs");
  int rc = check_epilogue_pointers(out, ldo, out_f32, resid, ldr, "conv3x3");
  if (rc) return rc;
  IgemmParams p;
  memset(&p, 0, sizeof(p));
  const int Ho = strided ? H / 2 : H, Wo = strided ? Wd / 2 : Wd;
  set_tile_shape(p, Wo, Ho, B);
  const uint64_t eb = 2;
  const int nkb = C / kBlockK;
  int nmaps = 0;
  int ntaps = 9;
  if (mode == 0 || folded) {
    rc = make_tmap_4d(&p.tmA[0], X, C, Wd, H, B, C * eb, (uint64_t)Wd * C * eb, (uint64_t)H * Wd * C * eb, kBlockK,
                      p.TW, p.TH, p.TB);
    if (rc) return rc;
    nmaps = 1;
    if (mode == 0) {
      for (int t = 0; t < 9; ++t)
        p.seg[t] = ASeg{0, static_cast<int16_t>(t % 3 - 1), static_cast<int16_t>(t / 3 - 1), static_cast<int16_t>(nkb), 0};
    } else {
      const int py = (mode - 3) >> 1, px = (mode - 3) & 1;
      ntaps = 4;
      for (int t = 0; t < 4; ++t)
        p.seg[t] = ASeg{0, static_cast<int16_t>((t & 1) - 1 + px), static_cast<int16_t>((t >> 1) - 1 + py), static_cast<int16_t>(nkb), 0};
    }
  } else {
    for (int py = 0; py < 2; ++py)
      for (int px = 0; px < 2; ++px) {
        const uint8_t* base = reinterpret_cast<const uint8_t*>(X) + (static_cast<uint64_t>(py) * Wd + px) * C * eb;
        rc = make_tmap_4d(&p.tmA[py * 2 + px], base, C, Wo, Ho, B, 2ull * C * eb, 2ull * Wd * C * eb,
                          (uint64_t)H * Wd * C * eb, kBlockK, p.TW, p.TH, p.TB);
        if (rc) return rc;
      }
    nmaps = 4;
    for (int t = 0; t < 9; ++t) {
      const int ky = t / 3, kx = t % 3;
      int py, dy, px, dx;
      if (mode == 1) {
        py = (ky == 1) ? 0 : 1; dy = (ky == 0) ? -1 : 0;
        px = (kx == 1) ? 0 : 1; dx = (kx == 0) ? -1 : 0;
      } else {
        py = (ky == 1) ? 1 : 0; dy = (ky == 2) ? 1 : 0;
        px = (kx == 1) ? 1 : 0; dx = (kx == 2) ? 1 : 0;
      }
      p.seg[t] = ASeg{static_cast<int16_t>(py * 2 + px), static_cast<int16_t>(dx), static_cast<int16_t>(dy),
                      static_cast<int16_t>(nkb), 0};
    }
  }
  p.nseg = ntaps;
  p.kb_total = ntaps * nkb;
  const void* sk[2] = {skip1, skip2};
  const int sc[2] = {Cs1, Cs2};
  for (int i = 0; i < 2; ++i) {
    if (!sk[i]) continue;
    rc = make_tmap_4d(&p.tmA[nmaps], sk[i], sc[i], Wo, Ho, B, sc[i] * eb, (uint64_t)Wo * sc[i] * eb,
                      (uint64_t)Ho * Wo * sc[i] * eb, kBlockK, p.TW, p.TH, p.TB);
    if (rc) return rc;
    p.seg[p.nseg] = ASeg{static_cast<int16_t>(nmaps), 0, 0, static_cast<int16_t>(sc[i] / kBlockK), 0};
    p.kb_total += sc[i] / kBlockK;
    ++p.nseg;
    ++nmaps;
  }
  for (int i = nmaps; i < kMaxA; ++i) p.tmA[i] = p.tmA[0];
  IgemmEpilogue e;
  e.bias = bias; e.bias_bstride = bias_bstride; e.rows_per_batch = Ho * Wo;
  e.resid = resid; e.ldr = ldr; e.out = out; e.ldo = ldo; e.out_f32 = out_f32; e.act = act; e.alpha = 1.f;
  e.out_parity = out_parity;
  return run_igemm(p, Wt, N, static_cast<long long>(p.kb_total) * kBlockK, ldw, e, bn, ksplit, workspace, ws_bytes,
                   reinterpret_cast<cudaStream_t>(stream));
}

}
```

### versatile-diffusion_b200/vdb200/_lib.py

```python
import ctypes as C
import os

LIB_PATH = os.environ.get("VDB200_LIB") or os.path.join(os.path.dirname(os.path.abspath(__file__)), "libvdb200.so")


class VdbError(RuntimeError):
    pass


if not os.path.exists(LIB_PATH):
    raise ImportError(
        f"{LIB_PATH} is missing: build it with `python -c 'import __graft_entry__ as g; g.build()'` "
        "(nvcc, sm_90a). vdb200 has no CPU / library fallback by design.")

lib = C.CDLL(LIB_PATH)

p, i, ll, f, sz = C.c_void_p, C.c_int, C.c_longlong, C.c_float, C.c_size_t

SIGNATURES = {
    "vdb_version": (C.c_char_p, []),
    "vdb_last_error": (C.c_char_p, []),
    "vdb_launch_count": (ll, []),
    "vdb_reset_launch_count": (None, []),
    "vdb_num_sms": (i, []),
    "vdb_ddim_cfg_step": (i, [p, p, p, p, p, p, f, f, p, p, p, ll, p]),
    "vdb_axpby_f32": (i, [p, p, f, f, p, ll, p]),
    "vdb_add_int": (i, [p, i, p]),
    "vdb_lincomb4_f32": (i, [p, p, p, p, f, f, f, f, p, ll, p]),
    "vdb_gemm_bf16": (i, [p, ll, ll, ll, p, ll, ll, p, ll, ll, p, ll, ll, p, ll, p, ll, i, i, f, i, i, p, sz, p]),
    "vdb_igemm_last_plan": (i, [C.POINTER(i), i]),
    "vdb_gemm_ln_bf16":(i, [p, ll, ll, ll, p, ll, ll, p, p, ll, p, ll, i, p, ll, i, i, f, p, i, p, p, p, i, p]),
    "vdb_gemm_skinny_fits": (i, [i, ll]),
    "vdb_gemm_skinny_bf16": (i, [p, i, ll, ll, p, ll, ll, p, ll, ll, p, ll, p, ll, p, ll, i, p]),
    "vdb_conv3x3_bf16": (i, [p, i, i, i, i, i, p, i, ll, p, i, p, i, p, ll, p, ll, p, ll, i, i, i, i, p, sz, p]),
    "vdb_attention_dk_pad": (i, [i]),
    "vdb_attention_dv_pad": (i, [i]),
    "vdb_attention_bf16": (i, [p, ll, i, p, ll, i, p, ll, p, ll, i, i, i, i, i, i, i, f, i, p]),
    "vdb_attention_varlen_bf16": (i, [p, ll, i, p, ll, i, p, ll, p, ll, i, i, i, i, i, i, i, f, i, p, p]),
    "vdb_groupnorm_nsplit": (i, [i, i]),
    "vdb_groupnorm_scratch_floats": (ll, [i, i]),
    "vdb_groupnorm_nhwc": (i, [p, i, p, i, i, i, i, p, p, f, i, p, p, p]),
    "vdb_layernorm": (i, [p, ll, i, p, p, f, p, p]),
    "vdb_norm_last_plan": (i, [C.POINTER(i), i]),
    "vdb_upsample2x_nhwc": (i, [p, i, i, i, i, p, p]),
    "vdb_interleave2x2_nhwc": (i, [p, i, i, i, i, p, p]),
    "vdb_clip_to_u8_hwc": (i, [p, i, i, i, p, p]),
    "vdb_resample_h_u8": (i, [p, i, i, i, i, p, p, i, p, p]),
    "vdb_resample_v_crop_norm": (i, [p, i, i, i, p, p, i, i, i, i, C.POINTER(f), C.POINTER(f), p, p]),
    "vdb_im2col3x3_small": (i, [p, i, i, i, i, i, f, f, p, p]),
    "vdb_permute_f32": (i, [p, i, i, ll, i, f, f, i, p, p]),
    "vdb_gaussian_sample": (i, [p, p, i, ll, f, p, p]),
    "vdb_cast_f32_bf16": (i, [p, p, ll, p]),
    "vdb_cast_bf16_f32": (i, [p, p, ll, p]),
    "vdb_pointwise_small": (i, [p, ll, i, i, p, p, f, p, p]),
    "vdb_timestep_embedding": (i, [p, p, i, i, f, p, p]),
    "vdb_linear_small": (i, [p, i, i, p, i, p, i, i, p, p]),
    "vdb_softmax_rows": (i, [p, ll, i, ll, f, p, p]),
    "vdb_clip_text_embed": (i, [p, p, p, i, i, i, i, p, p]),
    "vdb_patchify": (i, [p, i, i, i, i, i, p, p]),
    "vdb_vit_assemble": (i, [p, p, p, p, i, i, i, i, p, p]),
    "vdb_scale_by_row_norm": (i, [p, p, p, i, i, i, i, p, p]),
    "vdb_affine_act_rows": (i, [p, ll, i, p, p, i, p, p]),
    "vdb_pack_conv_weight": (i, [p, i, i, i, i, p, ll, ll, p]),
    "vdb_pack_geglu": (i, [p, p, i, i, p, p, p]),
    "vdb_pad_heads": (i, [p, i, i, i, i, p, p]),
    "vdb_textdec_gemv": (i, [p, i, ll, ll, p, p, f, p, ll, ll, p, i, i, p, ll, p]),
    "vdb_textdec_attention": (i, [p, ll, p, ll, p, p, i, i, i, p, f, p, ll, p]),
    "vdb_textdec_embed": (i, [p, i, p, p, i, p, i, i, p, i, i, p, p]),
    "vdb_textdec_sample": (i, [p, i, i, ll, f, p, p, i, p, i, p, i, p, p, p, i, i, p, p]),
}

for _name, (_res, _args) in SIGNATURES.items():
    _fn = getattr(lib, _name)
    _fn.restype = _res
    _fn.argtypes = _args


_TRACE = bool(os.environ.get("VDB_TRACE"))


def check(status: int, what: str = "") -> None:
    if _TRACE:
        import sys
        import torch
        print(f"[vdb] {what} ...", file=sys.stderr, flush=True)
        torch.cuda.synchronize()
        print(f"[vdb] {what} done", file=sys.stderr, flush=True)
    if status != 0:
        msg = lib.vdb_last_error().decode("utf-8", "replace")
        raise VdbError(f"vdb200 {what} failed with status {status}: {msg}")
```

### versatile-diffusion_b200/vdb200/ops.py

```python
import ctypes
import math
import os

import torch

from ._lib import lib, check

ACT_NONE, ACT_SILU, ACT_GELU, ACT_QUICK_GELU, ACT_GEGLU = 0, 1, 2, 3, 4
BF16 = torch.bfloat16


def _stream():
    return torch.cuda.current_stream().cuda_stream


def _ptr(t):
    return 0 if t is None else t.data_ptr()


def _need(t, dtype, name, rows_ok=False):
    if t is None:
        return
    if not t.is_cuda:
        raise ValueError(f"{name}: vdb200 kernels need CUDA tensors (no CPU fallback)")
    if t.dtype != dtype:
        raise TypeError(f"{name}: expected {dtype}, got {t.dtype}")
    if rows_ok and t.dim() == 2 and t.stride(1) == 1:
        return
    if not t.is_contiguous():
        raise ValueError(f"{name}: must be contiguous")


_workspace = {}
WORKSPACE_BYTES = 160 << 20


def _scratch_key(device):
    dev = device.index if device.index is not None else torch.cuda.current_device()
    sid = torch.cuda.current_stream(dev).cuda_stream
    owner = _scratch_owner.setdefault(dev, sid)
    if torch.cuda.is_current_stream_capturing():
        sid = owner
    return (dev, sid)


_scratch_owner = {}


def workspace(device):
    key = _scratch_key(device)
    w = _workspace.get(key)
    if w is None:
        if torch.cuda.is_current_stream_capturing():
            raise RuntimeError("split-K workspace must exist before CUDA-graph capture (run one eager step first)")
        w = torch.empty(WORKSPACE_BYTES // 4, dtype=torch.float32, device=device)
        _workspace[key] = w
    return w


_PROFILE = None


class _Span(object):
    __slots__ = ("name", "flops", "nbytes", "e0", "e1")

    def __init__(self, name, flops, nbytes):
        self.name, self.flops, self.nbytes = name, flops, nbytes

    def __enter__(self):
        if _PROFILE is not None:
            self.e0 = torch.cuda.Event(enable_timing=True)
            self.e1 = torch.cuda.Event(enable_timing=True)
            self.e0.record()
        return self

    def __exit__(self, *exc):
        if _PROFILE is not None:
            self.e1.record()
            _PROFILE.append(self)
        return False


def profile_start():
    global _PROFILE
    _PROFILE = []


def profile_stop():
    global _PROFILE
    spans, _PROFILE = _PROFILE, None
    torch.cuda.synchronize()
    out = {}
    for sp in spans or []:
        d = out.setdefault(sp.name, {"ms": 0.0, "launches": 0, "flops": 0.0, "bytes": 0.0})
        d["ms"] += sp.e0.elapsed_time(sp.e1)
        d["launches"] += 1
        d["flops"] += sp.flops
        d["bytes"] += sp.nbytes
    return out


_RECORD = None


def record_start():
    global _RECORD
    _RECORD = []


def record_stop():
    global _RECORD
    rec, _RECORD = _RECORD, None
    return rec or []


def replay(records):
    for fn, cargs, _keep, _flops in records:
        check(fn(*cargs, _stream()), "replay")


_gn_scratch_buf = {}


def _gn_scratch(device, nfloats):
    key = _scratch_key(device)
    buf = _gn_scratch_buf.get(key)
    if buf is None or buf.numel() < nfloats:
        if buf is not None and torch.cuda.is_current_stream_capturing():
            raise RuntimeError("GroupNorm scratch must be sized before CUDA-graph capture (run one eager step first)")
        buf = torch.zeros(max(int(nfloats), 1 << 20), dtype=torch.float32, device=device)
        _gn_scratch_buf[key] = buf
    return buf


def launch_count():
    return int(lib.vdb_launch_count())


def reset_launch_count():
    lib.vdb_reset_launch_count()


def ddim_cfg_step(e_uncond, e_cond, x, coef, scale, x_prev=None, pred_x0=None, noise=None,
                  temperature=1.0, step_idx=None, x_prev_dup=None):
    for n, t in (("e_uncond", e_uncond), ("e_cond", e_cond), ("x", x), ("noise", noise), ("coef", coef)):
        _need(t, torch.float32, n)
    if x_prev is None:
        x_prev = torch.empty_like(x)
    if step_idx is not None:
        _need(step_idx, torch.int32, "step_idx")
    check(lib.vdb_ddim_cfg_step(_ptr(e_uncond), _ptr(e_cond), _ptr(x), _ptr(noise), _ptr(coef), _ptr(step_idx),
                                float(scale), float(temperature), _ptr(x_prev), _ptr(x_prev_dup), _ptr(pred_x0), x.numel(),
                                _stream()),
          "ddim_cfg_step")
    return x_prev, pred_x0


def axpby(x, z, a, b, out=None):
    _need(x, torch.float32, "x"); _need(z, torch.float32, "z")
    if out is None:
        out = torch.empty_like(x)
    check(lib.vdb_axpby_f32(_ptr(x), _ptr(z), float(a), float(b), _ptr(out), x.numel(), _stream()), "axpby")
    return out


def lincomb4(xs, cs, out=None):
    assert 1 <= len(xs) <= 4 and len(xs) == len(cs)
    for t in xs:
        _need(t, torch.float32, "x")
    if out is None:
        out = torch.empty_like(xs[0])
    ptrs = [_ptr(t) for t in xs] + [0] * (4 - len(xs))
    coef = [float(c) for c in cs] + [0.0] * (4 - len(cs))
    check(lib.vdb_lincomb4_f32(ptrs[0], ptrs[1], ptrs[2], ptrs[3], coef[0], coef[1], coef[2], coef[3], _ptr(out),
                               xs[0].numel(), _stream()), "lincomb4")
    return out


def add_int(t, delta):
    _need(t, torch.int32, "counter")
    check(lib.vdb_add_int(_ptr(t), int(delta), _stream()), "add_int")


def _skinny_rows():
    return int(os.environ.get("VDB_SKINNY", "0"))


def gemm(a, w, bias=None, resid=None, out=None, act=ACT_NONE, a2=None, out_dtype=BF16, alpha=1.0,
         bias_bstride=0, rows_per_batch=1, bn=0, ksplit=0):
    _need(a, BF16, "a", True); _need(w, BF16, "w", True); _need(a2, BF16, "a2", True); _need(bias, torch.float32, "bias")
    _need(resid, BF16, "resid", True)
    M, K = a.shape
    N = w.shape[0]
    K2 = a2.shape[1] if a2 is not None else 0
    assert w.shape[1] == K + K2, (w.shape, K, K2)
    n_out = N // 2 if act == ACT_GEGLU else N
    if out is None:
        out = torch.empty((M, n_out), dtype=out_dtype, device=a.device)
    _need(out, out_dtype, "out", True)
    smax = _skinny_rows()
    if act == ACT_NONE and alpha == 1.0 and out_dtype == BF16 and bn == 0 and ksplit == 0 and smax > 0:
        if M <= smax and (bias_bstride == 0 or rows_per_batch == 1) and lib.vdb_gemm_skinny_fits(M, K + K2):
            check(lib.vdb_gemm_skinny_bf16(_ptr(a), M, K, a.stride(0), _ptr(a2), K2, a2.stride(0) if a2 is not None else 0,
                                           _ptr(w), N, w.stride(0), _ptr(bias), int(bias_bstride), _ptr(resid),
                                           resid.stride(0) if resid is not None else 0, _ptr(out), out.stride(0), 0, _stream()),
                  "gemm_skinny_bf16")
            return out
        if N <= smax and M > N and a2 is None and bias is None and resid is None and lib.vdb_gemm_skinny_fits(N, K):
            check(lib.vdb_gemm_skinny_bf16(_ptr(w), N, K, w.stride(0), None, 0, 0, _ptr(a), M, a.stride(0), None, 0, None, 0,
                                           _ptr(out), out.stride(0), 1, _stream()), "gemm_skinny_bf16")
            return out
    ws, ws_bytes = None, 0
    if ksplit != 1 and M <= 8192:
        ws, ws_bytes = workspace(a.device), WORKSPACE_BYTES
    cargs = (_ptr(a), M, K, a.stride(0), _ptr(a2), K2, a2.stride(0) if a2 is not None else 0,
             _ptr(w), N, w.stride(0), _ptr(bias), int(bias_bstride), int(rows_per_batch),
             _ptr(resid), resid.stride(0) if resid is not None else 0, _ptr(out), out.stride(0),
             1 if out_dtype == torch.float32 else 0, int(act), float(alpha), int(bn), int(ksplit),
             _ptr(ws), ws_bytes)
    with _Span("gemm", 2.0 * M * N * (K + K2), 2.0 * (M * (K + K2) + N * (K + K2) + M * n_out)):
        check(lib.vdb_gemm_bf16(*cargs, _stream()), "gemm_bf16")
    if _RECORD is not None:
        _RECORD.append((lib.vdb_gemm_bf16, cargs, (a, a2, w, bias, resid, out, ws), 2.0 * M * N * (K + K2)))
    return out


IGEMM_PLAN_FIELDS = ("bn", "stages", "mode", "ksplit", "grid", "tiles_m", "tiles_n", "nfast", "chunked")


def igemm_last_plan():
    buf = (ctypes.c_int * len(IGEMM_PLAN_FIELDS))()
    n = lib.vdb_igemm_last_plan(buf, len(buf))
    assert n == len(IGEMM_PLAN_FIELDS), n
    return dict(zip(IGEMM_PLAN_FIELDS, buf))


class LnFold(object):

    def __init__(self, stats, parts, dim, eps):
        self.stats, self.parts, self.dim, self.eps = stats, int(parts), int(dim), float(eps)


def ln_stats_buffer(rows, width, device):
    assert width % 32 == 0
    return torch.empty((2 * ((width + 63) // 64), rows, 2), dtype=torch.float32, device=device)


def gemm_ln(a, w, bias=None, resid=None, out=None, act=ACT_NONE, ln=None, colsum=None, on_cols=False, rowbias=None,
            stats_out=None, bn=0):
    _need(a, BF16, "a", True); _need(w, BF16, "w", True); _need(bias, torch.float32, "bias"); _need(resid, BF16, "resid", True)
    _need(colsum, torch.float32, "colsum"); _need(rowbias, torch.float32, "rowbias"); _need(stats_out, torch.float32, "stats_out")
    M, K = a.shape
    N = w.shape[0]
    assert w.shape[1] == K, (w.shape, K)
    n_out = N // 2 if act == ACT_GEGLU else N
    if out is None:
        out = torch.empty((M, n_out), dtype=BF16, device=a.device)
    _need(out, BF16, "out", True)
    st = None
    if ln is not None:
        st = ln.stats
        _need(st, torch.float32, "ln.stats")
        assert st.dim() == 3 and st.shape[0] >= ln.parts and st.shape[2] == 2, (tuple(st.shape), ln.parts)
    parts = ctypes.c_int(0)
    if stats_out is not None:
        assert stats_out.dim() == 3 and stats_out.shape[0] >= 2 * ((N + 63) // 64) and stats_out.shape[1] == M and stats_out.shape[2] == 2, \
            (tuple(stats_out.shape), N, M)
    cargs = (_ptr(a), M, K, a.stride(0), _ptr(w), N, w.stride(0), _ptr(bias), _ptr(resid),
             resid.stride(0) if resid is not None else 0, _ptr(out), out.stride(0), int(act),
             _ptr(st), st.shape[1] if st is not None else 0, ln.parts if ln is not None else 0, ln.dim if ln is not None else 0,
             ln.eps if ln is not None else 0.0, _ptr(colsum), 1 if on_cols else 0, _ptr(rowbias), _ptr(stats_out),
             ctypes.addressof(parts) if stats_out is not None else None, int(bn))
    with _Span("gemm", 2.0 * M * N * K, 2.0 * (M * K + N * K + M * n_out)):
        check(lib.vdb_gemm_ln_bf16(*cargs, _stream()), "gemm_ln_bf16")
    if _RECORD is not None:
        _RECORD.append((lib.vdb_gemm_ln_bf16, cargs, (a, w, bias, resid, out, st, colsum, rowbias, stats_out, parts), 2.0 * M * N * K))
    return (out, parts.value) if stats_out is not None else out


def conv3x3(x, w, bias=None, resid=None, out=None, mode=0, skip1=None, skip2=None, act=ACT_NONE,
            out_dtype=BF16, bias_bstride=0, bn=0, ksplit=0):
    _need(x, BF16, "x"); _need(w, BF16, "w"); _need(bias, torch.float32, "bias")
    _need(resid, BF16, "resid"); _need(skip1, BF16, "skip1"); _need(skip2, BF16, "skip2")
    B, H, W, Cc = x.shape
    N = w.shape[0]
    Ho, Wo = (H // 2, W // 2) if mode in (1, 2) else (H, W)
    cs1 = skip1.shape[-1] if skip1 is not None else 0
    cs2 = skip2.shape[-1] if skip2 is not None else 0
    ntaps = 4 if mode >= 3 else 9
    assert w.shape[1] == ntaps * Cc + cs1 + cs2, (w.shape, Cc, cs1, cs2, mode)
    if out is None:
        out = torch.empty((B, Ho, Wo, N), dtype=out_dtype, device=x.device)
    M = B * Ho * Wo
    ws, ws_bytes = None, 0
    if ksplit != 1 and M <= 8192:
        ws, ws_bytes = workspace(x.device), WORKSPACE_BYTES
    ktot = ntaps * Cc + cs1 + cs2
    cargs = (_ptr(x), B, H, W, Cc, int(mode), _ptr(w), N, w.stride(0), _ptr(skip1), cs1,
             _ptr(skip2), cs2, _ptr(bias), int(bias_bstride), _ptr(resid),
             resid.shape[-1] if resid is not None else 0, _ptr(out), out.shape[-1],
             1 if out_dtype == torch.float32 else 0, int(act), int(bn), int(ksplit), _ptr(ws), ws_bytes)
    with _Span("conv3x3", 2.0 * M * N * ktot, 2.0 * (B * H * W * Cc + M * (cs1 + cs2) + N * ktot + M * N)):
        check(lib.vdb_conv3x3_bf16(*cargs, _stream()), "conv3x3_bf16")
    if _RECORD is not None:
        _RECORD.append((lib.vdb_conv3x3_bf16, cargs, (x, w, skip1, skip2, bias, resid, out, ws), 2.0 * M * N * ktot))
    return out


def attention_pads(d_head):
    dk, dv = lib.vdb_attention_dk_pad(d_head), lib.vdb_attention_dv_pad(d_head)
    if dk < 0 or dv < 0:
        raise ValueError(f"d_head {d_head} unsupported by the attention kernel")
    return dk, dv


def attention(q, k, vt, out, B, H, Nq, Nk, d_head, scale=None, q_col0=0, k_col0=0, causal=False,
              q_bstride=0, kv_bstride=0, kv_len=None):
    _need(q, BF16, "q", True); _need(k, BF16, "k", True); _need(vt, BF16, "vt", True); _need(out, BF16, "out", True)
    _need(kv_len, torch.int32, "kv_len")
    if scale is None:
        scale = d_head ** -0.5
    args = (_ptr(q), q.stride(0), int(q_col0), _ptr(k), k.stride(0), int(k_col0), _ptr(vt), vt.stride(0), _ptr(out), out.stride(0),
            B, H, Nq, Nk, int(q_bstride), int(kv_bstride), d_head, float(scale), 1 if causal else 0)
    with _Span("attention", 4.0 * B * H * Nq * Nk * d_head, 2.0 * B * H * d_head * (2 * Nq + 2 * Nk)):
        if kv_len is None:
            check(lib.vdb_attention_bf16(*args, _stream()), "attention_bf16")
        else:
            check(lib.vdb_attention_varlen_bf16(*args, _ptr(kv_len), _stream()), "attention_varlen_bf16")
    return out


def groupnorm(x1, gamma, beta, eps, act=ACT_NONE, x2=None, out=None, groups=32):
    _need(x1, BF16, "x1"); _need(x2, BF16, "x2"); _need(gamma, torch.float32, "gamma"); _need(beta, torch.float32, "beta")
    B = x1.shape[0]
    C1 = x1.shape[-1]
    C2 = x2.shape[-1] if x2 is not None else 0
    HW = x1.numel() // (B * C1)
    if out is None:
        out = torch.empty(x1.shape[:-1] + (C1 + C2,), dtype=BF16, device=x1.device)
    partial = _gn_scratch(x1.device, lib.vdb_groupnorm_scratch_floats(B, HW))
    with _Span("groupnorm", 0.0, 2.0 * 3 * B * HW * (C1 + C2)):
        check(lib.vdb_groupnorm_nhwc(_ptr(x1), C1, _ptr(x2), C2, B, HW, groups, _ptr(gamma), _ptr(beta), float(eps),
                                     int(act), _ptr(partial), _ptr(out), _stream()), "groupnorm_nhwc")
    return out


def layernorm(x, gamma, beta, eps=1e-5, out=None):
    _need(x, BF16, "x"); _need(gamma, torch.float32, "gamma"); _need(beta, torch.float32, "beta")
    C = x.shape[-1]
    rows = x.numel() // C
    if out is None:
        out = torch.empty_like(x)
    with _Span("layernorm", 0.0, 2.0 * 2 * rows * C):
        check(lib.vdb_layernorm(_ptr(x), rows, C, _ptr(gamma), _ptr(beta), float(eps), _ptr(out), _stream()), "layernorm")
    return out


NORM_PLAN_FIELDS = ("family", "t0", "t1", "G", "S", "nsplit", "grid_x", "grid_y", "grid_z")
NORM_FAMILIES = {0: None, 1: "gn_bundle", 2: "gn_fused", 3: "gn_stats_apply", 4: "ln_rg", 5: "ln_warp"}


def norm_last_plan():
    buf = (ctypes.c_int * len(NORM_PLAN_FIELDS))()
    n = lib.vdb_norm_last_plan(buf, len(buf))
    assert n == len(NORM_PLAN_FIELDS), n
    plan = dict(zip(NORM_PLAN_FIELDS, buf))
    plan["family"] = NORM_FAMILIES[plan["family"]]
    return plan


def affine_silu_rows(x, gamma, beta, act=ACT_SILU, out=None):
    _need(x, BF16, "x"); _need(gamma, torch.float32, "gamma"); _need(beta, torch.float32, "beta")
    rows, n = x.shape
    if out is None:
        out = torch.empty_like(x)
    check(lib.vdb_affine_act_rows(_ptr(x), rows, n, _ptr(gamma), _ptr(beta), int(act), _ptr(out), _stream()), "affine_act_rows")
    return out


def pack_conv_weight(w, out=None, col0=0):
    _need(w, torch.float32, "w")
    Cout, Cin, kh, kw = w.shape
    if out is None:
        out = torch.empty((Cout, col0 + kh * kw * Cin), dtype=BF16, device=w.device)
    check(lib.vdb_pack_conv_weight(_ptr(w), Cout, Cin, kh, kw, _ptr(out), out.stride(0), col0, _stream()), "pack_conv_weight")
    return out


def pack_geglu(w, b=None):
    _need(w, torch.float32, "w")
    n2, K = w.shape[0] // 2, w.shape[1]
    wo = torch.empty((2 * n2, K), dtype=BF16, device=w.device)
    bo = torch.empty(2 * n2, dtype=torch.float32, device=w.device) if b is not None else None
    if b is not None:
        _need(b, torch.float32, "b")
    check(lib.vdb_pack_geglu(_ptr(w), _ptr(b) if b is not None else None, n2, K, _ptr(wo), _ptr(bo) if bo is not None else None,
                             _stream()), "pack_geglu")
    return wo, bo


def pad_heads(w, H, d, dpad):
    _need(w, torch.float32, "w")
    out = torch.empty((H * dpad, w.shape[1]), dtype=BF16, device=w.device)
    check(lib.vdb_pad_heads(_ptr(w), H, d, dpad, w.shape[1], _ptr(out), _stream()), "pad_heads")
    return out


def upsample2x(x, out=None):
    _need(x, BF16, "x")
    B, H, W, C = x.shape
    if out is None:
        out = torch.empty((B, 2 * H, 2 * W, C), dtype=BF16, device=x.device)
    check(lib.vdb_upsample2x_nhwc(_ptr(x), B, H, W, C, _ptr(out), _stream()), "upsample2x")
    return out


def interleave2x2(src, out=None):
    _need(src, BF16, "src")
    _, B, H, W, C = src.shape
    if out is None:
        out = torch.empty((B, 2 * H, 2 * W, C), dtype=BF16, device=src.device)
    check(lib.vdb_interleave2x2_nhwc(_ptr(src), B, H, W, C, _ptr(out), _stream()), "interleave2x2")
    return out


def upsample2x_conv3x3_folded(x, wf, bias=None):
    B, H, W, _ = x.shape
    N = wf.shape[1]
    if N % 32 == 0 and os.environ.get("VDB_UPFOLD_DIRECT", "1") != "0" and os.environ.get("VDB_EPI_TMA", "1") != "0" \
            and os.environ.get("VDB_IGEMM_SPEC", "1") != "0":
        out = torch.empty((B, 2 * H, 2 * W, N), dtype=BF16, device=x.device)
        for par in range(4):
            conv3x3(x, wf[par], bias=bias, out=out, mode=7 + par, ksplit=1)
        return out
    parts = torch.empty((4, B, H, W, N), dtype=BF16, device=x.device)
    for par in range(4):
        conv3x3(x, wf[par], bias=bias, out=parts[par], mode=3 + par, ksplit=1)
    return interleave2x2(parts)


def im2col3x3_small(x, kpad=64, in_scale=1.0, in_shift=0.0, out=None):
    _need(x, torch.float32, "x")
    B, H, W, Cin = x.shape
    if out is None:
        out = torch.empty((B * H * W, kpad), dtype=BF16, device=x.device)
    check(lib.vdb_im2col3x3_small(_ptr(x), B, H, W, Cin, kpad, float(in_scale), float(in_shift), _ptr(out), _stream()),
          "im2col3x3_small")
    return out


def nchw_to_nhwc(x, mul=1.0, add=0.0, out=None):
    _need(x, torch.float32, "x")
    B, C = x.shape[:2]
    HW = x.numel() // (B * C)
    if out is None:
        out = torch.empty((B,) + tuple(x.shape[2:]) + (C,), dtype=torch.float32, device=x.device)
    check(lib.vdb_permute_f32(_ptr(x), B, C, HW, 1, float(mul), float(add), 0, _ptr(out), _stream()), "permute")
    return out


def nhwc_to_nchw(x, mul=1.0, add=0.0, clamp01=False, out=None):
    _need(x, torch.float32, "x")
    B, C = x.shape[0], x.shape[-1]
    HW = x.numel() // (B * C)
    if out is None:
        out = torch.empty((B, C) + tuple(x.shape[1:-1]), dtype=torch.float32, device=x.device)
    check(lib.vdb_permute_f32(_ptr(x), B, C, HW, 0, float(mul), float(add), 1 if clamp01 else 0, _ptr(out), _stream()),
          "permute")
    return out


def to_bf16(x, out=None):
    _need(x, torch.float32, "x")
    if out is None:
        out = torch.empty(x.shape, dtype=BF16, device=x.device)
    check(lib.vdb_cast_f32_bf16(_ptr(x), _ptr(out), x.numel(), _stream()), "cast")
    return out


def to_f32(x, out=None):
    _need(x, BF16, "x")
    if out is None:
        out = torch.empty(x.shape, dtype=torch.float32, device=x.device)
    check(lib.vdb_cast_bf16_f32(_ptr(x), _ptr(out), x.numel(), _stream()), "cast")
    return out


def pointwise_small(x, w, bias=None, pre_mul=1.0, out=None):
    _need(x, torch.float32, "x"); _need(w, torch.float32, "w"); _need(bias, torch.float32, "bias")
    cout, cin = w.shape
    npix = x.numel() // cin
    if out is None:
        out = torch.empty(x.shape[:-1] + (cout,), dtype=torch.float32, device=x.device)
    check(lib.vdb_pointwise_small(_ptr(x), npix, cin, cout, _ptr(w), _ptr(bias), float(pre_mul), _ptr(out), _stream()),
          "pointwise_small")
    return out


def gaussian_sample(moments, noise=None, post_mul=1.0, out=None):
    _need(moments, torch.float32, "moments"); _need(noise, torch.float32, "noise")
    C = moments.shape[-1] // 2
    npix = moments.numel() // (2 * C)
    if out is None:
        out = torch.empty(moments.shape[:-1] + (C,), dtype=torch.float32, device=moments.device)
    check(lib.vdb_gaussian_sample(_ptr(moments), _ptr(noise), C, npix, float(post_mul), _ptr(out), _stream()),
          "gaussian_sample")
    return out


def timestep_embedding(ts, dim, max_period=10000, step_idx=None, batch=None, out=None):
    _need(ts, torch.int64, "timesteps")
    B = batch if step_idx is not None else ts.shape[0]
    if out is None:
        out = torch.empty((B, dim), dtype=torch.float32, device=ts.device)
    nlp = torch.tensor(-math.log(max_period), dtype=torch.float32).item()
    check(lib.vdb_timestep_embedding(_ptr(ts), _ptr(step_idx), B, dim, nlp, _ptr(out), _stream()), "timestep_embedding")
    return out


def linear_small(x, w, bias=None, act_in=ACT_NONE, act_out=ACT_NONE, out=None):
    _need(x, torch.float32, "x"); _need(w, BF16, "w"); _need(bias, torch.float32, "bias")
    M, K = x.shape
    N = w.shape[0]
    if out is None:
        out = torch.empty((M, N), dtype=torch.float32, device=x.device)
    check(lib.vdb_linear_small(_ptr(x), M, K, _ptr(w), N, _ptr(bias), int(act_in), int(act_out), _ptr(out), _stream()),
          "linear_small")
    return out


def softmax_rows(x, scale=1.0, out=None):
    _need(x, BF16, "x")
    n = x.shape[-1]
    rows = x.numel() // n
    if out is None:
        out = torch.empty_like(x)
    check(lib.vdb_softmax_rows(_ptr(x), rows, n, x.stride(-2) if x.dim() > 1 else n, float(scale), _ptr(out), _stream()),
          "softmax_rows")
    return out


def to_uint8_hwc(images):
    _need(images, torch.float32, "images")
    n, ch, H, W = images.shape
    assert ch == 3
    out = torch.empty((n, H, W, 3), dtype=torch.uint8, device=images.device)
    check(lib.vdb_clip_to_u8_hwc(_ptr(images), n, H, W, _ptr(out), _stream()), "clip_to_u8_hwc")
    return out


def clip_preprocess_device(images, tables, size, mean, std):
    import ctypes
    _need(images, torch.float32, "images")
    n, _, H, W = images.shape
    nw, nh = tables["nw"], tables["nh"]
    u8 = torch.empty((n, H, W, 3), dtype=torch.uint8, device=images.device)
    check(lib.vdb_clip_to_u8_hwc(_ptr(images), n, H, W, _ptr(u8), _stream()), "clip_to_u8_hwc")
    if tables["h"] is not None:
        hb, hk = tables["h"]
        mid = torch.empty((n, H, nw, 3), dtype=torch.uint8, device=images.device)
        check(lib.vdb_resample_h_u8(_ptr(u8), n, H, W, nw, _ptr(hb), _ptr(hk), hk.shape[1], _ptr(mid), _stream()), "resample_h_u8")
    else:
        mid = u8
    out = torch.empty((n, 3, size, size), dtype=torch.float32, device=images.device)
    vb, vk = tables["v"] if tables["v"] is not None else (None, None)
    m3, s3 = (ctypes.c_float * 3)(*mean), (ctypes.c_float * 3)(*std)
    check(lib.vdb_resample_v_crop_norm(_ptr(mid), n, H, nw, _ptr(vb), _ptr(vk), 0 if vk is None else vk.shape[1],
                                       (nh - size) // 2, (nw - size) // 2, size, m3, s3, _ptr(out), _stream()),
          "resample_v_crop_norm")
    return out


def clip_text_embed(tokens, tok_emb, pos_emb, Lp):
    _need(tokens, torch.int64, "tokens"); _need(tok_emb, torch.float32, "tok_emb"); _need(pos_emb, torch.float32, "pos_emb")
    B, L = tokens.shape
    C = tok_emb.shape[1]
    x = torch.empty((B, Lp, C), dtype=BF16, device=tokens.device)
    check(lib.vdb_clip_text_embed(_ptr(tokens), _ptr(tok_emb), _ptr(pos_emb), B, L, Lp, C, _ptr(x), _stream()), "clip_text_embed")
    return x


def patchify(pixels, patch, kpad):
    _need(pixels, torch.float32, "pixels")
    B, Cin, H, W = pixels.shape
    assert H == W
    g = H // patch
    y = torch.empty((B * g * g, kpad), dtype=BF16, device=pixels.device)
    check(lib.vdb_patchify(_ptr(pixels), B, Cin, H, patch, kpad, _ptr(y), _stream()), "patchify")
    return y


def vit_assemble(patches, cls, pos, B, L, Lp, tok_scale=None):
    _need(patches, BF16, "patches"); _need(cls, torch.float32, "cls"); _need(pos, torch.float32, "pos")
    _need(tok_scale, torch.float32, "tok_scale")
    C = patches.shape[1]
    x = torch.empty((B, Lp, C), dtype=BF16, device=patches.device)
    check(lib.vdb_vit_assemble(_ptr(patches), _ptr(cls), _ptr(pos), _ptr(tok_scale), B, L, Lp, C, _ptr(x), _stream()), "vit_assemble")
    return x


def scale_by_row_norm(z, L, idx=None, row_scale=None):
    _need(z, BF16, "z"); _need(idx, torch.int32, "idx"); _need(row_scale, torch.float32, "row_scale")
    B, Lp, C = z.shape
    out = torch.empty((B, L, C), dtype=torch.float32, device=z.device)
    check(lib.vdb_scale_by_row_norm(_ptr(z), _ptr(idx), _ptr(row_scale), B, L, Lp, C, _ptr(out), _stream()), "scale_by_row_norm")
    return out


ACT_GELU_TANH = 5
ACT_TANH = 6


def textdec_gemv(x, w, out, bias=None, ln=None, act=ACT_NONE, accumulate=False):
    _need(x, torch.float32, "x", rows_ok=True); _need(w, BF16, "w", rows_ok=True); _need(out, torch.float32, "out", rows_ok=True)
    _need(bias, torch.float32, "bias")
    g, b, eps = ln if ln is not None else (None, None, 0.0)
    _need(g, torch.float32, "ln_gamma"); _need(b, torch.float32, "ln_beta")
    R, K = x.shape
    N = w.shape[0]
    check(lib.vdb_textdec_gemv(_ptr(x), R, K, x.stride(0), _ptr(g), _ptr(b), float(eps), _ptr(w), N, w.stride(0), _ptr(bias),
                               int(act), int(bool(accumulate)), _ptr(out), out.stride(0), _stream()), "textdec_gemv")
    return out


def textdec_attention(qkv, mem, kcache, vcache, step, out, scale=0.125):
    for n, t in (("qkv", qkv), ("mem", mem), ("out", out)):
        _need(t, torch.float32, n, rows_ok=True)
    _need(kcache, torch.float32, "kcache"); _need(vcache, torch.float32, "vcache"); _need(step, torch.int32, "step")
    R, H, T, _ = kcache.shape
    check(lib.vdb_textdec_attention(_ptr(qkv), qkv.stride(0), _ptr(mem), mem.stride(0), _ptr(kcache), _ptr(vcache), R, H, T,
                                    _ptr(step), float(scale), _ptr(out), out.stride(0), _stream()), "textdec_attention")
    return out


def textdec_embed(tokens, step, wte, wpe, emb, out, pos_offset=1):
    _need(tokens, torch.int32, "tokens"); _need(step, torch.int32, "step")
    for n, t in (("wte", wte), ("wpe", wpe), ("emb", emb), ("out", out)):
        _need(t, torch.float32, n)
    R, D = out.shape
    check(lib.vdb_textdec_embed(_ptr(tokens), tokens.stride(0), _ptr(step), _ptr(wte), wte.shape[0], _ptr(wpe), wpe.shape[0],
                                int(pos_offset), _ptr(emb), R, D, _ptr(out), _stream()), "textdec_embed")
    return out


def textdec_sample(logits, tokens, done, lengths, step, temperature=1.0, seed=None, uniforms=None, forced=None, eos=50259,
                   max_len=30, record=None):
    _need(logits, torch.float32, "logits", rows_ok=True)
    _need(tokens, torch.int32, "tokens"); _need(done, torch.int32, "done"); _need(lengths, torch.int32, "lengths")
    _need(step, torch.int32, "step"); _need(seed, torch.int64, "seed"); _need(uniforms, torch.float64, "uniforms")
    _need(forced, torch.int32, "forced"); _need(record, torch.float32, "record")
    R, V = logits.shape
    check(lib.vdb_textdec_sample(_ptr(logits), R, V, logits.stride(0), float(temperature), _ptr(seed), _ptr(uniforms),
                                 uniforms.stride(0) if uniforms is not None else 0, _ptr(forced),
                                 forced.stride(0) if forced is not None else 0, _ptr(tokens), tokens.stride(0), _ptr(done),
                                 _ptr(lengths), _ptr(step), int(eos), int(max_len), _ptr(record), _stream()), "textdec_sample")
```

Baseline: 4.648.

## Add ping-pong warpgroup schedule to TMA-epilogue implicit GEMM with register rebalancing

Adds a ping-pong schedule for the TMA-store epilogue modes of the implicit GEMM. Each consumer warpgroup computes a full 128-row tile as two 64-row slabs, alternating tiles with the other warpgroup and handing off mainloop turns through named barriers, so one group's epilogue overlaps the other's MMA. Producer warps drop registers and consumers raise theirs via setmaxnreg, and a fourth producer-side warpgroup is added. It also allows GEGLU at BN 128 by loading two 64-column halves of the packed weight, which gives more tiles for small problems. The cost is doubled accumulator registers, more template instantiations, and extra barrier synchronisation, and the LN-stats prefetch is disabled on the ping-pong path.

```diff
diff --git a/include/vdb200.h b/include/vdb200.h
--- a/include/vdb200.h
+++ b/include/vdb200.h
@@ -33,6 +33,8 @@
                   size_t ws_bytes, void* stream);
 
 int vdb_igemm_last_plan(int* out, int n);
+
+int vdb_igemm_last_schedule(void);
 
 int vdb_gemm_ln_bf16(const void* A, long long M, long long K, long long lda, const void* W, long long N, long long ldw,
                      const float* bias, const void* resid, long long ldr, void* out, long long ldo, int act,
diff --git a/versatile-diffusion_b200/csrc/common.cuh b/versatile-diffusion_b200/csrc/common.cuh
--- a/versatile-diffusion_b200/csrc/common.cuh
+++ b/versatile-diffusion_b200/csrc/common.cuh
@@ -154,6 +154,14 @@
 #pragma unroll
   for (int i = 0; i < R; ++i) asm volatile("" : "+f"(d[i])::"memory");
 }
+
+template <uint32_t R>
+VDB_DEVINL void setmaxnreg_inc() { asm volatile("setmaxnreg.inc.sync.aligned.u32 %0;" ::"n"(R)); }
+template <uint32_t R>
+VDB_DEVINL void setmaxnreg_dec() { asm volatile("setmaxnreg.dec.sync.aligned.u32 %0;" ::"n"(R)); }
+
+VDB_DEVINL void named_bar_sync(int id, int threads) { asm volatile("bar.sync %0, %1;" ::"r"(id), "r"(threads) : "memory"); }
+VDB_DEVINL void named_bar_arrive(int id, int threads) { asm volatile("bar.arrive %0, %1;" ::"r"(id), "r"(threads) : "memory"); }
 
 VDB_DEVINL unsigned long long gtime() {
   unsigned long long t;
diff --git a/versatile-diffusion_b200/csrc/igemm.cu b/versatile-diffusion_b200/csrc/igemm.cu
--- a/versatile-diffusion_b200/csrc/igemm.cu
+++ b/versatile-diffusion_b200/csrc/igemm.cu
@@ -1,5 +1,7 @@
 #include "common.cuh"
 #include "host_util.h"
+
+#include <type_traits>
 
 namespace vdb {
 
@@ -75,14 +77,24 @@
   }
 }
 
-template <int BN, int STAGES, int EW, int MODE>
-__global__ void __launch_bounds__(32 + 32 * EW, 1) igemm_kernel(const __grid_constant__ IgemmParams p) {
+__host__ __device__ constexpr int igemm_threads(int mode, int ew) { return mode >= 3 ? 32 * ew + 128 : 32 * ew + 32; }
+__host__ __device__ constexpr bool igemm_sched_ok(int bn, int mode, int sched) {
+  return sched == 0 ? !((mode == 4 || mode == 6) && bn == 128) : (mode >= 3 && bn <= 160);
+}
+constexpr int kProducerRegs = 40, kConsumerRegs = 232;
+
+template <int BN, int STAGES, int EW, int MODE, int SCHED>
+__global__ void __launch_bounds__(igemm_threads(MODE, EW), 1) igemm_kernel(const __grid_constant__ IgemmParams p) {
   constexpr bool kTmaEpi = MODE >= 3;
   constexpr bool kGegluEpi = MODE == 4 || MODE == 6;
   constexpr bool kLnIn = MODE == 5 || MODE == 6;
   constexpr bool kStatsOut = MODE == 7;
+  static_assert(igemm_sched_ok(BN, MODE, SCHED), "ping-pong needs a TMA-store epilogue and BN <= 160; GEGLU at BN 128 needs it");
+  constexpr bool kPP = SCHED == 1;
+  constexpr int kSlabs = kPP ? 2 : 1;
+  constexpr bool kGeglu128 = kGegluEpi && BN == 128;
+  constexpr int kTabFloats = (kLnIn ? 2 : 1) * BN;
   constexpr int kNumEpiWarps = EW;
-  constexpr int kNumEpiThreads = EW * 32;
   constexpr int kWPQ = EW / 4;
   static_assert(EW == 8, "two consumer warpgroups of 64 rows each");
   constexpr uint32_t kBBytes = BN * kBlockK * 2;
@@ -103,17 +115,22 @@
   uint64_t* full_bar = reinterpret_cast<uint64_t*>(smem + kRegion + EW * 4096);
   uint64_t* empty_bar = full_bar + STAGES;
   uint64_t* acc_free = empty_bar + STAGES;
-  float* sbias = reinterpret_cast<float*>(acc_free + 2);
+  const int warp = threadIdx.x >> 5;
+  const int lane = threadIdx.x & 31;
+  const int wg = warp >> 2;
+  float* stab = reinterpret_cast<float*>(acc_free + 2);
+  float* sbias = stab + ((kPP && wg < 2) ? wg * kTabFloats : 0);
   float* slnx = sbias + BN;
   const uint32_t sbias_s = smem_u32(sbias), slnx_s = smem_u32(slnx);
   (void)slnx_s;
   if constexpr (kLnIn) {
-    if (reinterpret_cast<uint8_t*>(slnx + BN) > smem_raw + p.smem_bytes) __trap();
-  }
-  auto epi_bar_sync = [] { asm volatile("bar.sync 1, %0;" ::"n"(EW * 32) : "memory"); };
-
-  const int warp = threadIdx.x >> 5;
-  const int lane = threadIdx.x & 31;
+    if (reinterpret_cast<uint8_t*>(stab + kSlabs * kTabFloats) > smem_raw + p.smem_bytes) __trap();
+  }
+  auto epi_bar_sync = [&] {
+    if constexpr (kPP) named_bar_sync(2 + wg, 128);
+    else named_bar_sync(1, EW * 32);
+  };
+  const int tab_tid = kPP ? (threadIdx.x & 127) : static_cast<int>(threadIdx.x), tab_threads = kPP ? 128 : EW * 32;
 
   if (warp == EW && lane == 0) {
     for (int i = 0; i < kMaxA; ++i) tma_prefetch_desc(&p.tmA[i]);
@@ -123,7 +140,7 @@
   if (threadIdx.x == 0) {
     for (int s = 0; s < STAGES; ++s) {
       mbar_init(&full_bar[s], 1);
-      mbar_init(&empty_bar[s], kNumEpiWarps);
+      mbar_init(&empty_bar[s], kPP ? 4 : kNumEpiWarps);
     }
     mbar_init(acc_free, kNumEpiWarps);
     fence_barrier_init();
@@ -140,8 +157,9 @@
   const int t_first = p.chunked ? cta_id * per_cta : cta_id, t_step = p.chunked ? 1 : n_ctas;
   const int t_end = p.chunked ? min(num_tiles, t_first + per_cta) : num_tiles;
 
-  if (warp == EW) {
-    if (lane == 0) {
+  if (warp >= EW) {
+    if constexpr (kTmaEpi) setmaxnreg_dec<kProducerRegs>();
+    if (warp == EW && lane == 0) {
       uint32_t stage = 0, phase = 0;
       const bool flat = (p.tilesH == 1) && (p.tilesB == 1);
       const int step_m = t_step % unitsM, step_r = t_step / unitsM;
@@ -181,7 +199,13 @@
             mbar_arrive_expect_tx(&full_bar[stage], kStageBytes);
             tma_load_4d(smemA + stage * kABytes, &p.tmA[sg.tmap], &full_bar[stage],
                         sg.c0 + j * kBlockK, w0 + sg.dw, h0 + sg.dh, b0);
-            tma_load_2d(smemB + stage * kBBytes, &p.tmB, &full_bar[stage], kb * kBlockK, n0);
+            if constexpr (kGeglu128) {
+              const int nv = 256 * (n_idx >> 1) + 64 * (n_idx & 1);
+              tma_load_2d(smemB + stage * kBBytes, &p.tmB, &full_bar[stage], kb * kBlockK, nv);
+              tma_load_2d(smemB + stage * kBBytes + 64 * 128, &p.tmB, &full_bar[stage], kb * kBlockK, nv + 128);
+            } else {
+              tma_load_2d(smemB + stage * kBBytes, &p.tmB, &full_bar[stage], kb * kBlockK, n0);
+            }
             if (++stage == STAGES) { stage = 0; phase ^= 1; }
           }
           if (kb >= kb_end) break;
@@ -189,6 +213,7 @@
       }
     }
   } else {
+    if constexpr (kTmaEpi) setmaxnreg_inc<kConsumerRegs>();
     const int quarter = warp & 3;
     const int half = warp >> 2;
     const int r = quarter * 32 + lane;
@@ -204,19 +229,30 @@
       }
     };
     uint32_t ml_stage = 0, ml_phase = 0;
-    float acc[BN / 2];
-    auto mainloop = [&](int kb_begin, int kb_end) {
+    float acc[kSlabs][BN / 2];
+    auto mainloop = [&](int kb_begin, int kb_end, int it, bool hand_off) {
       const int g = warp >> 2;
 #pragma unroll
-      for (int i = 0; i < BN / 2; ++i) acc[i] = 0.f;
+      for (int s = 0; s < kSlabs; ++s)
+#pragma unroll
+        for (int i = 0; i < BN / 2; ++i) acc[s][i] = 0.f;
+      if constexpr (kPP) {
+        const int pos = it * p.kb_total;
+        ml_stage = static_cast<uint32_t>(pos % STAGES);
+        ml_phase = static_cast<uint32_t>((pos / STAGES) & 1);
+        if (it > 0) named_bar_sync(4 + g, 256);
+      }
       uint32_t prev = 0;
       for (int kb = kb_begin; kb < kb_end; ++kb) {
         mbar_wait(&full_bar[ml_stage], ml_phase);
         wgmma_fence();
-        const uint64_t adesc = make_desc_sw128(smem_u32(smemA + ml_stage * kABytes + g * (64 * 128)));
+        const uint32_t a_s = smem_u32(smemA + ml_stage * kABytes + (kPP ? 0 : g * (64 * 128)));
         const uint64_t bdesc = make_desc_sw128(smem_u32(smemB + ml_stage * kBBytes));
 #pragma unroll
-        for (int k = 0; k < kBlockK / 16; ++k) wgmma_ss<BN>(acc, adesc + 2 * k, bdesc + 2 * k, (kb > kb_begin || k > 0) ? 1u : 0u);
+        for (int k = 0; k < kBlockK / 16; ++k)
+#pragma unroll
+          for (int s = 0; s < kSlabs; ++s)
+            wgmma_ss<BN>(acc[s], make_desc_sw128(a_s + s * (64 * 128)) + 2 * k, bdesc + 2 * k, (kb > kb_begin || k > 0) ? 1u : 0u);
         wgmma_commit();
         if (kb > kb_begin) {
           wgmma_wait<1>();
@@ -226,8 +262,12 @@
         prev = ml_stage;
         if (++ml_stage == STAGES) { ml_stage = 0; ml_phase ^= 1; }
       }
+      if constexpr (kPP) {
+        if (hand_off) named_bar_arrive(4 + (g ^ 1), 256);
+      }
       wgmma_wait<0>();
-      wgmma_fence_regs(acc);
+#pragma unroll
+      for (int s = 0; s < kSlabs; ++s) wgmma_fence_regs(acc[s]);
       __syncwarp();
       if (lane == 0 && kb_end > kb_begin) mbar_arrive(&empty_bar[prev]);
       if constexpr (!kTmaEpi) {
@@ -235,8 +275,8 @@
         float* srow = sacc + (g * 64 + (warp & 3) * 16 + (lane >> 2)) * kAccStride + 2 * (lane & 3);
 #pragma unroll
         for (int j = 0; j < BN / 8; ++j) {
-          *reinterpret_cast<float2*>(srow + 8 * j) = make_float2(acc[4 * j], acc[4 * j + 1]);
-          *reinterpret_cast<float2*>(srow + 8 * kAccStride + 8 * j) = make_float2(acc[4 * j + 2], acc[4 * j + 3]);
+          *reinterpret_cast<float2*>(srow + 8 * j) = make_float2(acc[0][4 * j], acc[0][4 * j + 1]);
+          *reinterpret_cast<float2*>(srow + 8 * kAccStride + 8 * j) = make_float2(acc[0][4 * j + 2], acc[0][4 * j + 3]);
         }
         epi_bar_sync();
       }
@@ -266,17 +306,14 @@
     int unit_m = t_first % unitsM, rest = t_first / unitsM;
     const int nf_step_n = p.nfast ? t_step % p.tilesN : 0, nf_step_m = p.nfast ? t_step / p.tilesN : 0;
     int nf_n = p.nfast ? t_first % p.tilesN : 0, nf_m = p.nfast ? t_first / p.tilesN : 0;
-    const int e_row0 = (warp >> 2) * 64 + (warp & 3) * 16;
-    int e_tw[2], e_th[2], e_tb[2];
-#pragma unroll
-    for (int h = 0; h < 2; ++h) {
-      const int er = e_row0 + (lane >> 2) + 8 * h;
-      e_tw[h] = er % p.TW; e_th[h] = (er / p.TW) % p.TH; e_tb[h] = er / (p.TW * p.TH);
-    }
+    int e_row0[kSlabs];
+#pragma unroll
+    for (int sl = 0; sl < kSlabs; ++sl) e_row0[sl] = (kPP ? sl : (warp >> 2)) * 64 + (warp & 3) * 16;
     constexpr int kLnPre = 8;
-    float2 ln_pre[kLnIn ? kLnPre : 1];
+    constexpr bool kLnPrefetch = kLnIn && !kPP;
+    float2 ln_pre[kLnPrefetch ? kLnPre : 1];
     auto ln_prefetch = [&](int row) {
-      if constexpr (kLnIn) {
+      if constexpr (kLnPrefetch) {
         const bool ok = row < p.Wo;
         const int i0 = (lane >> 4) * kLnPre;
 #pragma unroll
@@ -286,8 +323,8 @@
                           : make_float2(0.f, 0.f);
       }
     };
-    if constexpr (kLnIn) {
-      if (!p.ln_on_cols && p.ln_parts <= 2 * kLnPre && t_first < t_end) ln_prefetch((t_first % unitsM) * kBlockM + e_row0 + (lane & 15));
+    if constexpr (kLnPrefetch) {
+      if (!p.ln_on_cols && p.ln_parts <= 2 * kLnPre && t_first < t_end) ln_prefetch((t_first % unitsM) * kBlockM + e_row0[0] + (lane & 15));
     }
     for (int t = t_first; t < t_end; t += t_step, ++it) {
       const int m_idx = p.nfast ? nf_m : unit_m;
@@ -304,6 +341,7 @@
       }
       unit_m += step_m; rest += step_r;
       if (unit_m >= unitsM) { unit_m -= unitsM; ++rest; }
+      if (kPP && (it & 1) != wg) continue;
       const int w = wt * p.TW + tw, h = ht * p.TH + th, b = bt * p.TB + tb;
       const bool row_ok = (w < p.Wo) && (h < p.Ho) && (b < p.Bo);
       const int gp = (b * p.Ho + h) * p.Wo + w;
@@ -325,12 +363,13 @@
       const bool bias_uniform = (MODE != 0) ? (p.bias != nullptr)
                                             : (p.bias && p.ksplit == 1 &&
                                                (p.bias_bstride == 0 || gp_first / p.rows_per_batch == gp_last / p.rows_per_batch));
+      auto tab_col = [&](int i) { return kGeglu128 ? 256 * (n_idx >> 1) + 64 * (n_idx & 1) + (i < 64 ? i : i + 64) : n0 + i; };
       if constexpr (kLnIn) {
         const float* key = reinterpret_cast<const float*>(static_cast<uintptr_t>(n0) + 1);
         if (key != sbias_src) {
           epi_bar_sync();
-          for (int i = threadIdx.x; i < BN; i += kNumEpiThreads) {
-            const int n = n0 + i;
+          for (int i = tab_tid; i < BN; i += tab_threads) {
+            const int n = tab_col(i);
             float a = 0.f, b = 0.f;
             if (n < p.N) {
               if (p.ln_on_cols) {
@@ -358,7 +397,7 @@
         const float* brow = p.bias + (p.bias_bstride ? static_cast<long long>(gp_first / p.rows_per_batch) * p.bias_bstride : 0) + n0;
         if (brow != sbias_src) {
           epi_bar_sync();
-          for (int i = threadIdx.x; i < BN; i += kNumEpiThreads) sbias[i] = (n0 + i < p.N) ? __ldg(brow + i) : 0.f;
+          for (int i = tab_tid; i < BN; i += tab_threads) sbias[i] = (tab_col(i) < p.N) ? __ldg(brow - n0 + tab_col(i)) : 0.f;
           epi_bar_sync();
           sbias_src = brow;
         }
@@ -379,56 +418,71 @@
         if (has_resid && f_first < f_nchunks) load_resid_fast(f_first, rr_first);
       }
 
-      int e_gp[2];
-      bool e_ok[2];
-#pragma unroll
-      for (int h = 0; h < 2; ++h) {
-        const int ew = wt * p.TW + e_tw[h], eh = ht * p.TH + e_th[h], eb = bt * p.TB + e_tb[h];
-        e_ok[h] = (ew < p.Wo) && (eh < p.Ho) && (eb < p.Bo);
-        e_gp[h] = (eb * p.Ho + eh) * p.Wo + ew;
-      }
-      float ln_a0[2] = {0.f, 0.f}, ln_a1[2] = {1.f, 1.f};
+      int e_gp[kSlabs][2];
+      bool e_ok[kSlabs][2];
+      auto epi_rows = [&] {
+#pragma unroll
+        for (int sl = 0; sl < kSlabs; ++sl)
+#pragma unroll
+          for (int h = 0; h < 2; ++h) {
+            const int er = e_row0[sl] + (lane >> 2) + 8 * h;
+            const int ew = wt * p.TW + er % p.TW, eh = ht * p.TH + (er / p.TW) % p.TH, eb = bt * p.TB + er / (p.TW * p.TH);
+            e_ok[sl][h] = (ew < p.Wo) && (eh < p.Ho) && (eb < p.Bo);
+            e_gp[sl][h] = (eb * p.Ho + eh) * p.Wo + ew;
+          }
+      };
+      if (kLnIn || !kTmaEpi) epi_rows();
+      float ln_a0[kSlabs][2], ln_a1[kSlabs][2];
+#pragma unroll
+      for (int sl = 0; sl < kSlabs; ++sl) { ln_a0[sl][0] = ln_a0[sl][1] = 0.f; ln_a1[sl][0] = ln_a1[sl][1] = 1.f; }
       if constexpr (kLnIn) {
         if (p.ln_on_cols) {
 #pragma unroll
-          for (int h = 0; h < 2; ++h) {
-            if (e_ok[h]) {
-              ln_a0[h] = __ldg(p.ln_colsum + e_gp[h]);
-              ln_a1[h] = p.ln_rowbias ? __ldg(p.ln_rowbias + e_gp[h]) : 0.f;
-            }
-          }
+          for (int sl = 0; sl < kSlabs; ++sl)
+#pragma unroll
+            for (int h = 0; h < 2; ++h) {
+              if (e_ok[sl][h]) {
+                ln_a0[sl][h] = __ldg(p.ln_colsum + e_gp[sl][h]);
+                ln_a1[sl][h] = p.ln_rowbias ? __ldg(p.ln_rowbias + e_gp[sl][h]) : 0.f;
+              }
+            }
         } else {
-          float su = 0.f, sq = 0.f;
-          if (p.ln_parts <= 2 * kLnPre) {
-#pragma unroll
-            for (int i = 0; i < kLnPre; ++i) { su += ln_pre[i].x; sq += ln_pre[i].y; }
-#pragma unroll
-            for (int i = 0; i < kLnPre; ++i) {
-              su += __shfl_sync(0xffffffffu, ln_pre[i].x, lane | 16);
-              sq += __shfl_sync(0xffffffffu, ln_pre[i].y, lane | 16);
-            }
-          } else {
-            const int row = m_idx * kBlockM + e_row0 + (lane & 15);
-            if (row < p.Wo) {
+#pragma unroll
+          for (int sl = 0; sl < kSlabs; ++sl) {
+            float su = 0.f, sq = 0.f;
+            if (kLnPrefetch && p.ln_parts <= 2 * kLnPre) {
+#pragma unroll
+              for (int i = 0; i < kLnPre; ++i) { su += ln_pre[i].x; sq += ln_pre[i].y; }
+#pragma unroll
+              for (int i = 0; i < kLnPre; ++i) {
+                su += __shfl_sync(0xffffffffu, ln_pre[i].x, lane | 16);
+                sq += __shfl_sync(0xffffffffu, ln_pre[i].y, lane | 16);
+              }
+            } else {
+              const int row = m_idx * kBlockM + e_row0[sl] + (lane & 15);
+              if (row < p.Wo) {
 #pragma unroll 8
-              for (int ch = 0; ch < p.ln_parts; ++ch) {
-                const float2 v = __ldg(reinterpret_cast<const float2*>(p.ln_stats) + static_cast<long long>(ch) * p.ln_mstat + row);
-                su += v.x; sq += v.y;
+                for (int ch = 0; ch < p.ln_parts; ++ch) {
+                  const float2 v = __ldg(reinterpret_cast<const float2*>(p.ln_stats) + static_cast<long long>(ch) * p.ln_mstat + row);
+                  su += v.x; sq += v.y;
+                }
               }
             }
-          }
-          const float mu = su * p.ln_inv_dim;
-          const float rs = rsqrtf(fmaxf(sq * p.ln_inv_dim - mu * mu, 0.f) + p.ln_eps);
-#pragma unroll
-          for (int h = 0; h < 2; ++h) {
-            ln_a0[h] = __shfl_sync(0xffffffffu, mu, (lane >> 2) + 8 * h);
-            ln_a1[h] = __shfl_sync(0xffffffffu, rs, (lane >> 2) + 8 * h);
+            const float mu = su * p.ln_inv_dim;
+            const float rs = rsqrtf(fmaxf(sq * p.ln_inv_dim - mu * mu, 0.f) + p.ln_eps);
+#pragma unroll
+            for (int h = 0; h < 2; ++h) {
+              ln_a0[sl][h] = __shfl_sync(0xffffffffu, mu, (lane >> 2) + 8 * h);
+              ln_a1[sl][h] = __shfl_sync(0xffffffffu, rs, (lane >> 2) + 8 * h);
+            }
           }
         }
-        if (!p.ln_on_cols && p.ln_parts <= 2 * kLnPre && t + t_step < t_end) ln_prefetch(unit_m * kBlockM + e_row0 + (lane & 15));
+        if (kLnPrefetch && !p.ln_on_cols && p.ln_parts <= 2 * kLnPre && t + t_step < t_end)
+          ln_prefetch(unit_m * kBlockM + e_row0[0] + (lane & 15));
       }
       VDB_TLE(4, it);
-      mainloop(ks * p.kb_per_split, min(p.kb_total, ks * p.kb_per_split + p.kb_per_split));
+      mainloop(ks * p.kb_per_split, min(p.kb_total, ks * p.kb_per_split + p.kb_per_split), it, t + t_step < t_end);
+      if (kTmaEpi && !kLnIn) epi_rows();
       VDB_TLE(5, it);
 
       auto geglu_tile = [&] {
@@ -471,146 +525,150 @@
       };
       if constexpr (kTmaEpi) {
         const uint32_t stg_s = smem_u32(sstage) + warp * 4096;
-        const int ow = wt * p.TW + (e_row0 % p.TW), oh = ht * p.TH + ((e_row0 / p.TW) % p.TH), ob = bt * p.TB + e_row0 / (p.TW * p.TH);
         constexpr int OUTC = kGegluEpi ? BN / 2 : BN;
         const int ochunks = kGegluEpi ? OUTC / 32 : f_nchunks;
         const int ocol0 = n_idx * OUTC;
         const int tq2 = 2 * (lane & 3);
-        const bool do_resid = (MODE == 3 || MODE == 7) && has_resid;
-        const uint32_t* rrow[2];
-#pragma unroll
-        for (int h = 0; h < 2; ++h)
-          rrow[h] = (do_resid && e_ok[h]) ? reinterpret_cast<const uint32_t*>(p.resid + static_cast<long long>(e_gp[h]) * p.ldr + ocol0 + tq2)
-                                          : nullptr;
-        auto load_resid = [&](int c, uint32_t (&rr)[2][4]) {
+#pragma unroll
+        for (int sl = 0; sl < kSlabs; ++sl) {
+          const int er0 = e_row0[sl];
+          const int ow = wt * p.TW + (er0 % p.TW), oh = ht * p.TH + ((er0 / p.TW) % p.TH), ob = bt * p.TB + er0 / (p.TW * p.TH);
+          const bool do_resid = (MODE == 3 || MODE == 7) && has_resid;
+          const uint32_t* rrow[2];
 #pragma unroll
           for (int h = 0; h < 2; ++h)
-#pragma unroll
-            for (int jj = 0; jj < 4; ++jj) rr[h][jj] = rrow[h] ? __ldg(rrow[h] + (c * 32 + 8 * jj) / 2) : 0u;
-        };
-        uint32_t rr[2][4];
-        if (do_resid) load_resid(0, rr);
-        float st_su[2][2] = {{0.f, 0.f}, {0.f, 0.f}}, st_sq[2][2] = {{0.f, 0.f}, {0.f, 0.f}};
-        (void)st_su; (void)st_sq;
-        float nrm[2];
-#pragma unroll
-        for (int h = 0; h < 2; ++h) nrm[h] = -ln_a1[h] * ln_a0[h];
-        (void)nrm;
-#pragma unroll
-        for (int c = 0; c < OUTC / 32; ++c) {
-          if (c >= ochunks) break;
-          float o[4][2][2];
-#pragma unroll
-          for (int jj = 0; jj < 4; ++jj) {
-            const int n = c * 32 + 8 * jj + tq2;
-            const float* va = acc + 4 * (4 * c + jj);
-            if constexpr (kGegluEpi) {
-              const float* vg = acc + 4 * (BN / 16 + 4 * c + jj);
-              if constexpr (kLnIn) {
-                const float2 sa = lds_f2(slnx_s + 4 * n), ca = lds_f2(sbias_s + 4 * n);
-                const float2 sg = lds_f2(slnx_s + 4 * (OUTC + n)), cg = lds_f2(sbias_s + 4 * (OUTC + n));
-#pragma unroll
-                for (int h = 0; h < 2; ++h) {
-                  o[jj][h][0] = fmaf(ln_a1[h], va[2 * h], fmaf(nrm[h], sa.x, ca.x)) * gelu_fast_f(fmaf(ln_a1[h], vg[2 * h], fmaf(nrm[h], sg.x, cg.x)));
-                  o[jj][h][1] = fmaf(ln_a1[h], va[2 * h + 1], fmaf(nrm[h], sa.y, ca.y)) * gelu_fast_f(fmaf(ln_a1[h], vg[2 * h + 1], fmaf(nrm[h], sg.y, cg.y)));
+            rrow[h] = (do_resid && e_ok[sl][h]) ? reinterpret_cast<const uint32_t*>(p.resid + static_cast<long long>(e_gp[sl][h]) * p.ldr + ocol0 + tq2)
+                                            : nullptr;
+          auto load_resid = [&](int c, uint32_t (&rr)[2][4]) {
+#pragma unroll
+            for (int h = 0; h < 2; ++h)
+#pragma unroll
+              for (int jj = 0; jj < 4; ++jj) rr[h][jj] = rrow[h] ? __ldg(rrow[h] + (c * 32 + 8 * jj) / 2) : 0u;
+          };
+          uint32_t rr[2][4];
+          if (do_resid) load_resid(0, rr);
+          float st_su[2][2] = {{0.f, 0.f}, {0.f, 0.f}}, st_sq[2][2] = {{0.f, 0.f}, {0.f, 0.f}};
+          (void)st_su; (void)st_sq;
+          float nrm[2];
+#pragma unroll
+          for (int h = 0; h < 2; ++h) nrm[h] = -ln_a1[sl][h] * ln_a0[sl][h];
+          (void)nrm;
+#pragma unroll
+          for (int c = 0; c < OUTC / 32; ++c) {
+            if (c >= ochunks) break;
+            float o[4][2][2];
+#pragma unroll
+            for (int jj = 0; jj < 4; ++jj) {
+              const int n = c * 32 + 8 * jj + tq2;
+              const float* va = acc[sl] + 4 * (4 * c + jj);
+              if constexpr (kGegluEpi) {
+                const float* vg = acc[sl] + 4 * (BN / 16 + 4 * c + jj);
+                if constexpr (kLnIn) {
+                  const float2 sa = lds_f2(slnx_s + 4 * n), ca = lds_f2(sbias_s + 4 * n);
+                  const float2 sg = lds_f2(slnx_s + 4 * (OUTC + n)), cg = lds_f2(sbias_s + 4 * (OUTC + n));
+#pragma unroll
+                  for (int h = 0; h < 2; ++h) {
+                    o[jj][h][0] = fmaf(ln_a1[sl][h], va[2 * h], fmaf(nrm[h], sa.x, ca.x)) * gelu_fast_f(fmaf(ln_a1[sl][h], vg[2 * h], fmaf(nrm[h], sg.x, cg.x)));
+                    o[jj][h][1] = fmaf(ln_a1[sl][h], va[2 * h + 1], fmaf(nrm[h], sa.y, ca.y)) * gelu_fast_f(fmaf(ln_a1[sl][h], vg[2 * h + 1], fmaf(nrm[h], sg.y, cg.y)));
+                  }
+                } else {
+                  const float2 ba = p.bias ? lds_f2(sbias_s + 4 * n) : make_float2(0.f, 0.f);
+                  const float2 bg = p.bias ? lds_f2(sbias_s + 4 * (OUTC + n)) : make_float2(0.f, 0.f);
+#pragma unroll
+                  for (int h = 0; h < 2; ++h) {
+                    o[jj][h][0] = (va[2 * h] + ba.x) * gelu_fast_f(vg[2 * h] + bg.x);
+                    o[jj][h][1] = (va[2 * h + 1] + ba.y) * gelu_fast_f(vg[2 * h + 1] + bg.y);
+                  }
+                }
+              } else if constexpr (kLnIn) {
+                if (p.ln_on_cols) {
+                  const float2 mu = lds_f2(slnx_s + 4 * n), rs = lds_f2(sbias_s + 4 * n);
+#pragma unroll
+                  for (int h = 0; h < 2; ++h) {
+                    o[jj][h][0] = fmaf(rs.x, fmaf(mu.x, -ln_a0[sl][h], va[2 * h]), ln_a1[sl][h]);
+                    o[jj][h][1] = fmaf(rs.y, fmaf(mu.y, -ln_a0[sl][h], va[2 * h + 1]), ln_a1[sl][h]);
+                  }
+                } else {
+                  const float2 sx = lds_f2(slnx_s + 4 * n), cx = lds_f2(sbias_s + 4 * n);
+#pragma unroll
+                  for (int h = 0; h < 2; ++h) {
+                    o[jj][h][0] = fmaf(ln_a1[sl][h], va[2 * h], fmaf(nrm[h], sx.x, cx.x));
+                    o[jj][h][1] = fmaf(ln_a1[sl][h], va[2 * h + 1], fmaf(nrm[h], sx.y, cx.y));
+                  }
                 }
               } else {
-                const float2 ba = p.bias ? lds_f2(sbias_s + 4 * n) : make_float2(0.f, 0.f);
-                const float2 bg = p.bias ? lds_f2(sbias_s + 4 * (OUTC + n)) : make_float2(0.f, 0.f);
+                const float2 bb = p.bias ? lds_f2(sbias_s + 4 * n) : make_float2(0.f, 0.f);
 #pragma unroll
                 for (int h = 0; h < 2; ++h) {
-                  o[jj][h][0] = (va[2 * h] + ba.x) * gelu_fast_f(vg[2 * h] + bg.x);
-                  o[jj][h][1] = (va[2 * h + 1] + ba.y) * gelu_fast_f(vg[2 * h + 1] + bg.y);
+                  o[jj][h][0] = va[2 * h] + bb.x;
+                  o[jj][h][1] = va[2 * h + 1] + bb.y;
                 }
               }
-            } else if constexpr (kLnIn) {
-              if (p.ln_on_cols) {
-                const float2 mu = lds_f2(slnx_s + 4 * n), rs = lds_f2(sbias_s + 4 * n);
-#pragma unroll
-                for (int h = 0; h < 2; ++h) {
-                  o[jj][h][0] = fmaf(rs.x, fmaf(mu.x, -ln_a0[h], va[2 * h]), ln_a1[h]);
-                  o[jj][h][1] = fmaf(rs.y, fmaf(mu.y, -ln_a0[h], va[2 * h + 1]), ln_a1[h]);
+            }
+            if (do_resid) {
+              uint32_t rn[2][4];
+              const bool more = c + 1 < ochunks;
+              if (more) load_resid(c + 1, rn);
+#pragma unroll
+              for (int h = 0; h < 2; ++h)
+#pragma unroll
+                for (int jj = 0; jj < 4; ++jj) {
+                  const float2 x = unpack_bf16x2(rr[h][jj]);
+                  o[jj][h][0] += x.x;
+                  o[jj][h][1] += x.y;
                 }
-              } else {
-                const float2 sx = lds_f2(slnx_s + 4 * n), cx = lds_f2(sbias_s + 4 * n);
-#pragma unroll
-                for (int h = 0; h < 2; ++h) {
-                  o[jj][h][0] = fmaf(ln_a1[h], va[2 * h], fmaf(nrm[h], sx.x, cx.x));
-                  o[jj][h][1] = fmaf(ln_a1[h], va[2 * h + 1], fmaf(nrm[h], sx.y, cx.y));
-                }
+              if (more) {
+#pragma unroll
+                for (int h = 0; h < 2; ++h)
+#pragma unroll
+                  for (int jj = 0; jj < 4; ++jj) rr[h][jj] = rn[h][jj];
               }
-            } else {
-              const float2 bb = p.bias ? lds_f2(sbias_s + 4 * n) : make_float2(0.f, 0.f);
-#pragma unroll
-              for (int h = 0; h < 2; ++h) {
-                o[jj][h][0] = va[2 * h] + bb.x;
-                o[jj][h][1] = va[2 * h + 1] + bb.y;
+            }
+            if constexpr (kStatsOut) {
+#pragma unroll
+              for (int h = 0; h < 2; ++h)
+#pragma unroll
+                for (int jj = 0; jj < 4; ++jj)
+#pragma unroll
+                  for (int e = 0; e < 2; ++e) {
+                    st_su[h][c & 1] += o[jj][h][e];
+                    st_sq[h][c & 1] = fmaf(o[jj][h][e], o[jj][h][e], st_sq[h][c & 1]);
+                  }
+            }
+            if (lane == 0) bulk_wait_read<3>();
+            __syncwarp();
+            const uint32_t box = stg_s + st_buf * 1024;
+            {
+              const int mi = lane >> 3, brow = (mi & 1) * 8 + (lane & 7);
+#pragma unroll
+              for (int u = 0; u < 2; ++u) {
+                const int unit = 2 * u + (mi >> 1);
+                stmatrix_x4(box + brow * 64 + ((unit ^ ((brow >> 1) & 3)) << 4),
+                            pack_bf16x2(o[2 * u][0][0], o[2 * u][0][1]), pack_bf16x2(o[2 * u][1][0], o[2 * u][1][1]),
+                            pack_bf16x2(o[2 * u + 1][0][0], o[2 * u + 1][0][1]), pack_bf16x2(o[2 * u + 1][1][0], o[2 * u + 1][1][1]));
               }
             }
-          }
-          if (do_resid) {
-            uint32_t rn[2][4];
-            const bool more = c + 1 < ochunks;
-            if (more) load_resid(c + 1, rn);
-#pragma unroll
-            for (int h = 0; h < 2; ++h)
-#pragma unroll
-              for (int jj = 0; jj < 4; ++jj) {
-                const float2 x = unpack_bf16x2(rr[h][jj]);
-                o[jj][h][0] += x.x;
-                o[jj][h][1] += x.y;
-              }
-            if (more) {
-#pragma unroll
-              for (int h = 0; h < 2; ++h)
-#pragma unroll
-                for (int jj = 0; jj < 4; ++jj) rr[h][jj] = rn[h][jj];
-            }
+            fence_proxy_async_smem();
+            __syncwarp();
+            if (lane == 0) {
+              tma_store_4d(&p.tmO, reinterpret_cast<const uint8_t*>(sstage) + warp * 4096 + st_buf * 1024, ocol0 + c * 32, ow, oh, ob);
+              bulk_commit();
+            }
+            st_buf = (st_buf + 1) & 3;
           }
           if constexpr (kStatsOut) {
 #pragma unroll
             for (int h = 0; h < 2; ++h)
 #pragma unroll
-              for (int jj = 0; jj < 4; ++jj)
-#pragma unroll
-                for (int e = 0; e < 2; ++e) {
-                  st_su[h][c & 1] += o[jj][h][e];
-                  st_sq[h][c & 1] = fmaf(o[jj][h][e], o[jj][h][e], st_sq[h][c & 1]);
-                }
+              for (int par = 0; par < 2; ++par) {
+                float su = st_su[h][par], sq = st_sq[h][par];
+                su += __shfl_xor_sync(0xffffffffu, su, 1); sq += __shfl_xor_sync(0xffffffffu, sq, 1);
+                su += __shfl_xor_sync(0xffffffffu, su, 2); sq += __shfl_xor_sync(0xffffffffu, sq, 2);
+                if ((lane & 3) == 0 && e_ok[sl][h])
+                  reinterpret_cast<float2*>(p.stats_out)[static_cast<long long>(n_idx * 2 + par) * (static_cast<long long>(p.Bo) * p.Ho * p.Wo) + e_gp[sl][h]] =
+                      make_float2(su, sq);
+              }
           }
-          if (lane == 0) bulk_wait_read<3>();
-          __syncwarp();
-          const uint32_t box = stg_s + st_buf * 1024;
-          {
-            const int mi = lane >> 3, brow = (mi & 1) * 8 + (lane & 7);
-#pragma unroll
-            for (int u = 0; u < 2; ++u) {
-              const int unit = 2 * u + (mi >> 1);
-              stmatrix_x4(box + brow * 64 + ((unit ^ ((brow >> 1) & 3)) << 4),
-                          pack_bf16x2(o[2 * u][0][0], o[2 * u][0][1]), pack_bf16x2(o[2 * u][1][0], o[2 * u][1][1]),
-                          pack_bf16x2(o[2 * u + 1][0][0], o[2 * u + 1][0][1]), pack_bf16x2(o[2 * u + 1][1][0], o[2 * u + 1][1][1]));
-            }
-          }
-          fence_proxy_async_smem();
-          __syncwarp();
-          if (lane == 0) {
-            tma_store_4d(&p.tmO, reinterpret_cast<const uint8_t*>(sstage) + warp * 4096 + st_buf * 1024, ocol0 + c * 32, ow, oh, ob);
-            bulk_commit();
-          }
-          st_buf = (st_buf + 1) & 3;
-        }
-        if constexpr (kStatsOut) {
-#pragma unroll
-          for (int h = 0; h < 2; ++h)
-#pragma unroll
-            for (int par = 0; par < 2; ++par) {
-              float su = st_su[h][par], sq = st_sq[h][par];
-              su += __shfl_xor_sync(0xffffffffu, su, 1); sq += __shfl_xor_sync(0xffffffffu, sq, 1);
-              su += __shfl_xor_sync(0xffffffffu, su, 2); sq += __shfl_xor_sync(0xffffffffu, sq, 2);
-              if ((lane & 3) == 0 && e_ok[h])
-                reinterpret_cast<float2*>(p.stats_out)[static_cast<long long>(n_idx * 2 + par) * (static_cast<long long>(p.Bo) * p.Ho * p.Wo) + e_gp[h]] =
-                    make_float2(su, sq);
-            }
         }
       } else if constexpr (MODE == 1) {
         uint4 rr[4];
@@ -814,25 +872,26 @@
   }
 }
 
-template <int BN, int STAGES, int EW, int MODE>
+template <int BN, int STAGES, int EW, int MODE, int SCHED = 0>
 static int launch_igemm(const IgemmParams& p0, int num_units, cudaStream_t stream) {
   constexpr bool kLn = MODE == 5 || MODE == 6;
+  constexpr int tables = SCHED ? 2 : 1;
   constexpr size_t ring = STAGES * (kABytes + BN * kBlockK * 2), acc = kBlockM * (BN + 4) * 4;
-  constexpr size_t need = (ring > acc ? ring : acc) + (2 * STAGES + 2) * 8 + BN * 4 + (kLn ? BN * 4 : 0) + EW * 4096;
+  constexpr size_t need = (ring > acc ? ring : acc) + (2 * STAGES + 2) * 8 + tables * (BN * 4 + (kLn ? BN * 4 : 0)) + EW * 4096;
   constexpr size_t smem = (need + 1024 <= 227 * 1024) ? need + 1024 : 227 * 1024;
   static_assert(need + 896 <= 227 * 1024, "igemm shared-memory budget");
-  constexpr int threads = 32 + 32 * EW;
+  constexpr int threads = igemm_threads(MODE, EW);
   IgemmParams p = p0;
   p.smem_bytes = static_cast<unsigned>(smem);
   static bool configured = false;
   if (!configured) {
-    VDB_CUDA_CHECK(cudaFuncSetAttribute(igemm_kernel<BN, STAGES, EW, MODE>, cudaFuncAttributeMaxDynamicSharedMemorySize,
+    VDB_CUDA_CHECK(cudaFuncSetAttribute(igemm_kernel<BN, STAGES, EW, MODE, SCHED>, cudaFuncAttributeMaxDynamicSharedMemorySize,
                                         static_cast<int>(smem)));
-    prefer_max_smem(igemm_kernel<BN, STAGES, EW, MODE>);
+    prefer_max_smem(igemm_kernel<BN, STAGES, EW, MODE, SCHED>);
     configured = true;
   }
   const int grid = std::min(num_units, num_sms());
-  VDB_CUDA_CHECK(launch_pdl(igemm_kernel<BN, STAGES, EW, MODE>, dim3(grid), dim3(threads), smem, stream, p));
+  VDB_CUDA_CHECK(launch_pdl(igemm_kernel<BN, STAGES, EW, MODE, SCHED>, dim3(grid), dim3(threads), smem, stream, p));
   count_launch();
   return VDB_OK;
 }
@@ -853,6 +912,7 @@
 
 constexpr int kPlanFields = 9;
 static thread_local int g_last_plan[kPlanFields] = {0};
+static thread_local int g_last_schedule = 0;
 
 static int check_epilogue_pointers(const void* out, long long ldo, int out_f32, const void* resid, long long ldr, const char* who) {
   if ((reinterpret_cast<uintptr_t>(out) & 15) || (resid && (reinterpret_cast<uintptr_t>(resid) & 15)))
@@ -916,7 +976,8 @@
     while (BN > 64 && tiles(BN) * 2 <= num_sms()) BN = (BN == 256) ? 160 : (BN == 160 ? 128 : 64);
   }
   if (BN != 64 && BN != 128 && BN != 160 && BN != 256) return set_error(VDB_ERR_INVALID, "igemm: bad BN");
-  if (e.act == ACT_GEGLU && (N % BN) != 0) return set_error(VDB_ERR_INVALID, "igemm: GEGLU needs N % 256 == 0");
+  if (e.act == ACT_GEGLU && (N % 256) != 0) return set_error(VDB_ERR_INVALID, "igemm: GEGLU needs N % 256 == 0");
+  if (e.act == ACT_GEGLU && BN != 256 && BN != 128) return set_error(VDB_ERR_INVALID, "igemm: GEGLU runs at BN 256 or 128");
   p.N = static_cast<int>(N);
   p.tilesN = static_cast<int>((N + BN - 1) / BN);
   p.bias = e.bias; p.bias_bstride = e.bias_bstride; p.rows_per_batch = e.rows_per_batch > 0 ? e.rows_per_batch : 1;
@@ -962,7 +1023,7 @@
     p.chunked = (chunked_mode != 0 && !p.nfast && p.ksplit == 1 && p.tilesN > 1 && units >= 3LL * grid) ? 1 : 0;
   }
   int rc = make_tmap_2d(&p.tmB, Wt, static_cast<uint64_t>(Ktot), static_cast<uint64_t>(N),
-                        static_cast<uint64_t>(ldw) * 2, kBlockK, BN);
+                        static_cast<uint64_t>(ldw) * 2, kBlockK, (e.act == ACT_GEGLU && BN == 128) ? 64 : BN);
   if (rc) return rc;
   const int num_tiles = mn_tiles * p.ksplit;
   static const int spec = [] { const char* ev = getenv("VDB_IGEMM_SPEC"); return (ev && ev[0] == '0') ? 0 : 1; }();
@@ -971,7 +1032,7 @@
                             (p.TB == 1 && (static_cast<long long>(p.Ho) * p.Wo == p.rows_per_batch ||
                                            (p.Ho == 1 && p.Bo == 1 && p.rows_per_batch % kBlockM == 0)));
   if (spec && p.ksplit == 1 && !e.out_f32 && one_bias_row) {
-    if (e.act == ACT_GEGLU && BN == 256) mode = 2;
+    if (e.act == ACT_GEGLU && (BN == 256 || BN == 128)) mode = 2;
     else if (e.act == ACT_NONE && e.alpha == 1.f && (N % 32) == 0) mode = 1;
   }
   static const int epi_tma = [] { const char* ev = getenv("VDB_EPI_TMA"); return (ev && ev[0] == '0') ? 0 : 1; }();
@@ -1001,36 +1062,32 @@
     if (ln_in && mode == 4 && e.ln_on_cols) return set_error(VDB_ERR_UNSUPPORTED, "igemm: GEGLU with column statistics");
     mode = st_out ? 7 : mode + 2;
   }
+  if (e.act == ACT_GEGLU && BN == 128 && mode != 4 && mode != 6)
+    return set_error(VDB_ERR_UNSUPPORTED, "igemm: GEGLU at BN 128 needs the TMA-store epilogue (bf16 out, aligned out, VDB_EPI_TMA != 0)");
+  const bool pp = mode >= 3 && BN <= 160 &&
+                  ((e.act == ACT_GEGLU && BN == 128) || num_tiles >= 3 * std::min(num_tiles, num_sms()));
   {
     const int stages = BN == 64 ? 8 : BN == 128 ? 6 : BN == 160 ? 5 : 4;
     const int plan[kPlanFields] = {BN, stages, mode, p.ksplit, std::min(num_tiles, num_sms()), tilesM, p.tilesN, p.nfast, p.chunked};
     for (int i = 0; i < kPlanFields; ++i) g_last_plan[i] = plan[i];
-  }
-  if (mode == 7) {
-    switch (BN) {
-      case 64: rc = launch_igemm<64, 8, 8, 7>(p, num_tiles, stream); break;
-      case 128: rc = launch_igemm<128, 6, 8, 7>(p, num_tiles, stream); break;
-      case 160: rc = launch_igemm<160, 5, 8, 7>(p, num_tiles, stream); break;
-      default: rc = launch_igemm<256, 4, 8, 7>(p, num_tiles, stream); break;
-    }
+    g_last_schedule = pp ? 1 : 0;
+  }
+  if (mode == 3 || mode == 5 || mode == 7) {
+    auto tma_mode = [&](auto mode_c) -> int {
+      constexpr int M = decltype(mode_c)::value;
+      switch (BN) {
+        case 64: return pp ? launch_igemm<64, 8, 8, M, 1>(p, num_tiles, stream) : launch_igemm<64, 8, 8, M, 0>(p, num_tiles, stream);
+        case 128: return pp ? launch_igemm<128, 6, 8, M, 1>(p, num_tiles, stream) : launch_igemm<128, 6, 8, M, 0>(p, num_tiles, stream);
+        case 160: return pp ? launch_igemm<160, 5, 8, M, 1>(p, num_tiles, stream) : launch_igemm<160, 5, 8, M, 0>(p, num_tiles, stream);
+        default: return launch_igemm<256, 4, 8, M, 0>(p, num_tiles, stream);
+      }
+    };
+    rc = mode == 3 ? tma_mode(std::integral_constant<int, 3>()) : mode == 5 ? tma_mode(std::integral_constant<int, 5>())
+                                                                            : tma_mode(std::integral_constant<int, 7>());
   } else if (mode == 6) {
-    rc = launch_igemm<256, 4, 8, 6>(p, num_tiles, stream);
-  } else if (mode == 5) {
-    switch (BN) {
-      case 64: rc = launch_igemm<64, 8, 8, 5>(p, num_tiles, stream); break;
-      case 128: rc = launch_igemm<128, 6, 8, 5>(p, num_tiles, stream); break;
-      case 160: rc = launch_igemm<160, 5, 8, 5>(p, num_tiles, stream); break;
-      default: rc = launch_igemm<256, 4, 8, 5>(p, num_tiles, stream); break;
-    }
+    rc = BN == 128 ? launch_igemm<128, 6, 8, 6, 1>(p, num_tiles, stream) : launch_igemm<256, 4, 8, 6>(p, num_tiles, stream);
   } else if (mode == 4) {
-    rc = launch_igemm<256, 4, 8, 4>(p, num_tiles, stream);
-  } else if (mode == 3) {
-    switch (BN) {
-      case 64: rc = launch_igemm<64, 8, 8, 3>(p, num_tiles, stream); break;
-      case 128: rc = launch_igemm<128, 6, 8, 3>(p, num_tiles, stream); break;
-      case 160: rc = launch_igemm<160, 5, 8, 3>(p, num_tiles, stream); break;
-      default: rc = launch_igemm<256, 4, 8, 3>(p, num_tiles, stream); break;
-    }
+    rc = BN == 128 ? launch_igemm<128, 6, 8, 4, 1>(p, num_tiles, stream) : launch_igemm<256, 4, 8, 4>(p, num_tiles, stream);
   } else if (mode == 2) {
     rc = launch_igemm<256, 4, 8, 2>(p, num_tiles, stream);
   } else if (mode == 1) {
@@ -1087,6 +1144,8 @@
   for (int i = 0; out && i < n && i < kPlanFields; ++i) out[i] = g_last_plan[i];
   return kPlanFields;
 }
+
+int vdb_igemm_last_schedule(void) { return g_last_schedule; }
 
 int vdb_gemm_bf16(const void* A, long long M, long long K, long long lda, const void* A2, long long K2,
                   long long lda2, const void* W, long long N, long long ldw, const float* bias,
diff --git a/versatile-diffusion_b200/vdb200/_lib.py b/versatile-diffusion_b200/vdb200/_lib.py
--- a/versatile-diffusion_b200/vdb200/_lib.py
+++ b/versatile-diffusion_b200/vdb200/_lib.py
@@ -29,6 +29,7 @@
     "vdb_lincomb4_f32": (i, [p, p, p, p, f, f, f, f, p, ll, p]),
     "vdb_gemm_bf16": (i, [p, ll, ll, ll, p, ll, ll, p, ll, ll, p, ll, ll, p, ll, p, ll, i, i, f, i, i, p, sz, p]),
     "vdb_igemm_last_plan": (i, [C.POINTER(i), i]),
+    "vdb_igemm_last_schedule": (i, []),
     "vdb_gemm_ln_bf16":(i, [p, ll, ll, ll, p, ll, ll, p, p, ll, p, ll, i, p, ll, i, i, f, p, i, p, p, p, i, p]),
     "vdb_gemm_skinny_fits": (i, [i, ll]),
     "vdb_gemm_skinny_bf16": (i, [p, i, ll, ll, p, ll, ll, p, ll, ll, p, ll, p, ll, p, ll, i, p]),
diff --git a/versatile-diffusion_b200/vdb200/ops.py b/versatile-diffusion_b200/vdb200/ops.py
--- a/versatile-diffusion_b200/vdb200/ops.py
+++ b/versatile-diffusion_b200/vdb200/ops.py
@@ -232,7 +232,7 @@
     buf = (ctypes.c_int * len(IGEMM_PLAN_FIELDS))()
     n = lib.vdb_igemm_last_plan(buf, len(buf))
     assert n == len(IGEMM_PLAN_FIELDS), n
-    return dict(zip(IGEMM_PLAN_FIELDS, buf))
+    return dict(zip(IGEMM_PLAN_FIELDS, buf), schedule=lib.vdb_igemm_last_schedule())
 
 
 class LnFold(object):
```

Result: faster. 4.820, median of 6 (+3.7%).
